# h3poteto/aws-global-accelerator-controller

Measured on NVIDIA H100. Metric: objects reconciled/sec at 10^6 Service+Ingress; change-set bit-exact vs Go ref, higher is better.
Workload: dtype u8/u32 (bytes and indices)

## Files before the change

aws-global-accelerator-controller_b200/csrc/gar_engine.cu:

```cuda

#include <cuda_runtime.h>
#include <unistd.h>

#include <cstdio>
#include <cstdlib>
#include <cstring>
#include <atomic>
#include <exception>
#include <functional>
#include <mutex>
#include <thread>
#include <string>
#include <vector>
#include <type_traits>
#include <utility>

#include "gar_pipeline.h"
#include "gar_shard.h"
#include "gar_delta.h"

#define GAR_VERSION_STRING "garecon 0.1.0 (sm_90a)"


template <class F>
__global__ void __launch_bounds__(256) k_for_each(const __grid_constant__ F f, u32 n) {
  u32 i = blockIdx.x * blockDim.x + threadIdx.x;
  if (i < n) f(i);
}

template <class F, int MINB>
__global__ void __launch_bounds__(256, MINB) k_for_each_warp(const __grid_constant__ F f, u32 n) {
  u32 i = blockIdx.x * blockDim.x + threadIdx.x;
  f(i, i < n);
}
__device__ __forceinline__ u32 smem_addr(const void *p) { return (u32)__cvta_generic_to_shared(p); }
__device__ __forceinline__ void mbar_init(u64 *bar, u32 count) {
  asm volatile("mbarrier.init.shared::cta.b64 [%0], %1;" ::"r"(smem_addr(bar)), "r"(count));
  asm volatile("fence.mbarrier_init.release.cluster;" ::: "memory");
}
__device__ __forceinline__ void mbar_expect_tx(u64 *bar, u32 bytes) {
  asm volatile("mbarrier.arrive.expect_tx.shared::cta.b64 _, [%0], %1;" ::"r"(smem_addr(bar)), "r"(bytes) : "memory");
}
__device__ __forceinline__ void tma_bulk_g2s(void *dst, const void *src, u32 bytes, u64 *bar) {
  asm volatile("cp.async.bulk.shared::cluster.global.mbarrier::complete_tx::bytes [%0], [%1], %2, [%3];" ::"r"(smem_addr(dst)), "l"(src), "r"(bytes),
               "r"(smem_addr(bar))
               : "memory");
}
__device__ __forceinline__ void mbar_wait(u64 *bar, u32 parity) {
  u32 done;
  do {
    asm volatile("{ .reg .pred p; mbarrier.try_wait.parity.shared::cta.b64 p, [%1], %2; selp.u32 %0, 1, 0, p; }" : "=r"(done) : "r"(smem_addr(bar)), "r"(parity) : "memory");
  } while (!done);
}
struct StagedView {
  const u8 *smem[2];
  const u8 *slab[2];
  u64 lo[2], hi[2];
  __device__ __forceinline__ Str operator()(int c, gar_str r) const {
    const u64 o = GAR_STR_OFF(r), n = GAR_STR_LEN(r);
    if (o >= lo[c] && o + n + 16 <= hi[c]) return Str{smem[c] + (o - lo[c]), (u32)n};
    return Str{slab[c] + o, (u32)n};
  }
};
template <class F>
__global__ void __launch_bounds__(256) k_for_each_staged(const __grid_constant__ F f, u32 n) {
  constexpr u32 STAGE_BYTES = F::kStageBytes;
  __shared__ alignas(128) u8 buf[F::kStageCols][STAGE_BYTES];
  __shared__ alignas(8) u64 bar;
  __shared__ u32 s_bytes[2];
  __shared__ u64 s_lo[2];
  const u32 r0 = blockIdx.x * blockDim.x, r1 = min(r0 + blockDim.x, n);
  if (threadIdx.x == 0) {
    mbar_init(&bar, 1);
    u32 total = 0;
    for (int c = 0; c < F::kStageCols; c++) {
      u64 lo = 0, hi = 0;
      u32 bytes = 0;
      const u8 *slab = f.stage_slab(c);
      if (f.stage_window(c, r0, r1, &lo, &hi) && hi > lo && (((uintptr_t)slab) & 15) == 0) {
        lo &= ~(u64)15;
        u64 span = ((hi - lo + 15) & ~(u64)15) + 16;
        if (span > STAGE_BYTES) span = STAGE_BYTES;
        bytes = (u32)span;
      }
      s_lo[c] = lo;
      s_bytes[c] = bytes;
      total += bytes;
    }
    mbar_expect_tx(&bar, total);
    for (int c = 0; c < F::kStageCols; c++)
      if (s_bytes[c]) tma_bulk_g2s(buf[c], f.stage_slab(c) + s_lo[c], s_bytes[c], &bar);
  }
  __syncthreads();
  StagedView view;
#pragma unroll
  for (int c = 0; c < 2; c++) {
    const bool on = c < F::kStageCols;
    view.smem[c] = on ? buf[c < F::kStageCols ? c : 0] : nullptr;
    view.slab[c] = on ? f.stage_slab(c) : nullptr;
    view.lo[c] = on ? s_lo[c] : 1;
    view.hi[c] = on ? s_lo[c] + s_bytes[c] : 0;
  }
  mbar_wait(&bar, 0);
  const u32 i = r0 + threadIdx.x;
  if (i < n) f.run(i, view);
}

template <class F>
__global__ void __launch_bounds__(256) k_for_each_dyn(const __grid_constant__ F f, const u32 *n_dev, u32 cap) {
  u32 n = *n_dev;
  if (n > cap) n = cap;
  u32 i = blockIdx.x * blockDim.x + threadIdx.x;
  if (i < n) f(i);
}
template <class F, int MINB>
__global__ void __launch_bounds__(256, MINB) k_for_each_warp_dyn(const __grid_constant__ F f, const u32 *n_dev, u32 cap) {
  u32 n = *n_dev;
  if (n > cap) n = cap;
  u32 i = blockIdx.x * blockDim.x + threadIdx.x;
  if (i < ((n + 31u) & ~31u)) f(i, i < n);
}
template <class... Fs>
struct FPack;
template <>
struct FPack<> {
  __device__ __forceinline__ void call(int, u32) const {}
};
template <class F, class... R>
struct FPack<F, R...> {
  F f;
  FPack<R...> rest;
  FPack(const F &f_, const R &...r) : f(f_), rest(r...) {}
  __device__ __forceinline__ void call(int k, u32 i) const {
    if (k == 0) f(i);
    else rest.call(k - 1, i);
  }
};
constexpr int MULTI_MAX = 8;
struct MultiRanges {
  u32 blk_end[MULTI_MAX], n[MULTI_MAX];
  int count;
};
template <class P>
__global__ void __launch_bounds__(256) k_for_each_multi(const __grid_constant__ P pack, const __grid_constant__ MultiRanges r) {
  int k = 0;
  while (k + 1 < r.count && blockIdx.x >= r.blk_end[k]) k++;
  u32 i = (blockIdx.x - (k ? r.blk_end[k - 1] : 0u)) * blockDim.x + threadIdx.x;
  if (i < r.n[k]) pack.call(k, i);
}

template <class F> struct MinBlocks { static constexpr int value = 2; };
template <> struct MinBlocks<FGaObj> { static constexpr int value = 4; };
template <> struct MinBlocks<FR53Pair> { static constexpr int value = 6; };
template <> struct MinBlocks<FR53Prepare> { static constexpr int value = 6; };

__global__ void k_fill32(u32 *p, u32 v, size_t n) {
  size_t i = (size_t)blockIdx.x * blockDim.x + threadIdx.x;
  size_t stride = (size_t)gridDim.x * blockDim.x;
  for (; i < n; i += stride) p[i] = v;
}

constexpr int SCAN_THREADS = 256;
constexpr int SCAN_ITEMS = 8;
constexpr int SCAN_TILE = SCAN_THREADS * SCAN_ITEMS;

__device__ __forceinline__ u32 warp_incl_scan(u32 v) {
  const unsigned lane = threadIdx.x & 31;
#pragma unroll
  for (int d = 1; d < 32; d <<= 1) {
    u32 t = __shfl_up_sync(0xffffffffu, v, d);
    if (lane >= (unsigned)d) v += t;
  }
  return v;
}
__device__ __forceinline__ u32 block_excl_scan(u32 v, u32 *total) {
  __shared__ u32 wsum[SCAN_THREADS / 32];
  __shared__ u32 wtot;
  const unsigned lane = threadIdx.x & 31, w = threadIdx.x >> 5;
  u32 inc = warp_incl_scan(v);
  if (lane == 31) wsum[w] = inc;
  __syncthreads();
  if (w == 0) {
    u32 s = lane < SCAN_THREADS / 32 ? wsum[lane] : 0;
    u32 si = warp_incl_scan(s);
    if (lane < SCAN_THREADS / 32) wsum[lane] = si - s;
    if (lane == SCAN_THREADS / 32 - 1) wtot = si;
  }
  __syncthreads();
  u32 r = wsum[w] + inc - v;
  *total = wtot;
  __syncthreads();
  return r;
}

__global__ void __launch_bounds__(SCAN_THREADS) k_scan_lookback(u32 *data, u32 n, unsigned long long *state, u32 *ticket) {
  __shared__ u32 s_tile, s_excl;
  if (threadIdx.x == 0) s_tile = atomicAdd(ticket, 1u);
  __syncthreads();
  const u32 tile = s_tile;
  const u32 base = tile * SCAN_TILE + threadIdx.x * SCAN_ITEMS;
  u32 v[SCAN_ITEMS];
  if (base + SCAN_ITEMS <= n) {
    const uint4 *q = reinterpret_cast<const uint4 *>(data + base);
    uint4 a = q[0], b = q[1];
    v[0] = a.x; v[1] = a.y; v[2] = a.z; v[3] = a.w;
    v[4] = b.x; v[5] = b.y; v[6] = b.z; v[7] = b.w;
  } else {
#pragma unroll
    for (int k = 0; k < SCAN_ITEMS; k++) v[k] = base + k < n ? data[base + k] : 0;
  }
  u32 s = 0;
#pragma unroll
  for (int k = 0; k < SCAN_ITEMS; k++) s += v[k];
  u32 total;
  u32 ex = block_excl_scan(s, &total);
  if (threadIdx.x < 32) {
    volatile unsigned long long *st = state;
    const unsigned lane = threadIdx.x;
    if (tile == 0) {
      if (lane == 0) {
        st[0] = (2ull << 62) | total;
        s_excl = 0;
      }
    } else {
      if (lane == 0) {
        st[tile] = (1ull << 62) | total;
        __threadfence();
      }
      u32 excl = 0;
      for (long long p = (long long)tile - 1;; p -= 32) {
        long long idx = p - (long long)lane;
        unsigned long long w = 2ull << 62;
        if (idx >= 0) {
          do {
            w = st[idx];
          } while ((w >> 62) == 0);
        }
        unsigned pm = __ballot_sync(0xffffffffu, (w >> 62) == 2);
        int first = __ffs(pm) - 1;
        u32 val = (first < 0 || (int)lane <= first) ? (u32)w : 0u;
#pragma unroll
        for (int off = 16; off > 0; off >>= 1) val += __shfl_down_sync(0xffffffffu, val, off);
        excl += val;
        if (first >= 0) break;
      }
      if (lane == 0) {
        st[tile] = (2ull << 62) | (u32)(excl + total);
        s_excl = excl;
      }
    }
  }
  __syncthreads();
  ex += s_excl;
  if (base + SCAN_ITEMS <= n) {
    uint4 a, b;
    a.x = ex; ex += v[0];
    a.y = ex; ex += v[1];
    a.z = ex; ex += v[2];
// ... 275 lines not shown
    for (int r = 0; r < 2; r++)
      for (int k = 0; k < GAR_SHARD_MAX_RANKS; k++) {
        if (peer_mapped[r][k]) cudaIpcCloseMemHandle(peer_ptr[r][k]);
        peer_mapped[r][k] = false;
        peer_ptr[r][k] = nullptr;
        peer_seen[r][k] = PeerHandle{};
      }
  }
  std::vector<HostResult *> free_results;
  float ms_h2d = 0;
  u32 launches = 0;
  u64 input_bytes = 0;
  bool timing = false;
  bool reprepare = false;
  bool no_orphans = false, allow_empty_cache = false;
  struct Mark {
    const char *name;
    cudaEvent_t a, b;
    u32 launches;
  };
  std::vector<Mark> marks;
  std::vector<cudaEvent_t> event_pool;
  size_t events_used = 0;
  int stage_depth = 0;
  u32 stage_launch0 = 0;
  std::vector<gar_stage_timing> last_timings;
  u64 last_counters[GAR_CTR_N] = {};
  cudaEvent_t new_event() {
    if (events_used == event_pool.size()) {
      cudaEvent_t ev;
      CK(cudaEventCreate(&ev));
      event_pool.push_back(ev);
    }
    return event_pool[events_used++];
  }
  void stage_begin(const char *name) {
    if (!timing || stage_depth++ > 0) return;
    Mark m{name, new_event(), new_event(), 0};
    CK(cudaEventRecord(m.a, stream));
    stage_launch0 = launches;
    marks.push_back(m);
  }
  void stage_end() {
    if (!timing || --stage_depth > 0) return;
    marks.back().launches = launches - stage_launch0;
    CK(cudaEventRecord(marks.back().b, stream));
  }

  void *dev_ensure(DBuf &b, size_t bytes) {
    bytes = (bytes + 255) & ~(size_t)255;
    if (b.cap < bytes) {
      if (capturing) throw CudaError{"internal: a buffer grew while a launch sequence was being recorded"};
      graph_drop();
      if (b.p) CK(cudaFree(b.p));
      b.p = nullptr;
      b.cap = 0;
      size_t want = bytes + bytes / 4;
      CK(cudaMalloc(&b.p, want));
      b.cap = want;
    }
    return b.p;
  }
  void *pin_ensure(DBuf &b, size_t bytes) {
    if (bytes < 64) bytes = 64;
    if (b.cap < bytes) {
      if (b.p) CK(cudaFreeHost(b.p));
      b.p = nullptr;
      b.cap = 0;
      size_t want = bytes + bytes / 4;
      CK(cudaMallocHost(&b.p, want));
      b.cap = want;
    }
    return b.p;
  }

  bool pack_tma = false;
  template <class F>
  void for_each(const char *name, u32 n, const F &f) {
    if (!n) return;
    stage_begin(name);
    if constexpr (std::is_same<F, FShPackRows>::value) {
      if (pack_tma) {
        k_shard_pack_rows<<<(n + 255) / 256, 256, 0, stream>>>(f, n);
        launches++;
        stage_end();
        return;
      }
    }
    k_for_each<F><<<(n + 255) / 256, 256, 0, stream>>>(f, n);
    launches++;
    stage_end();
  }
  template <class F>
  void for_each_warp(const char *name, u32 n, const F &f) {
    if (!n) return;
    stage_begin(name);
    k_for_each_warp<F, MinBlocks<F>::value><<<(n + 255) / 256, 256, 0, stream>>>(f, n);
    launches++;
    stage_end();
  }
  u32 hint_dport_cap = 0, hint_pair_cap = 0;
  u64 hint_ops_cap = 0;
  bool use_graphs = true;
  cudaGraphExec_t graph_exec = nullptr;
  u64 graph_sig = 0, seen_sig = 0;
  u32 graph_launches = 0, capture_launch0 = 0;
  bool capturing = false;
  void graph_drop() {
    if (graph_exec) cudaGraphExecDestroy(graph_exec);
    graph_exec = nullptr;
    graph_sig = seen_sig = 0;
  }
  int graph_begin(u64 sig) {
    if (!use_graphs || timing) return 0;
    if (graph_exec && graph_sig == sig) {
      CK(cudaGraphLaunch(graph_exec, stream));
      launches += graph_launches;
      return 2;
    }
    if (seen_sig != sig) {
      graph_drop();
      seen_sig = sig;
      return 0;
    }
    graph_drop();
    seen_sig = sig;
    CK(cudaStreamBeginCapture(stream, cudaStreamCaptureModeThreadLocal));
    capturing = true;
    capture_launch0 = launches;
    return 1;
  }
  void graph_end() {
    if (!capturing) return;
    capturing = false;
    cudaGraph_t g = nullptr;
    CK(cudaStreamEndCapture(stream, &g));
    cudaError_t ie = cudaGraphInstantiate(&graph_exec, g, 0);
    cudaGraphDestroy(g);
    if (ie != cudaSuccess) {
      graph_exec = nullptr;
      throw CudaError{std::string("cudaGraphInstantiate failed: ") + cudaGetErrorString(ie)};
    }
    graph_sig = seen_sig;
    graph_launches = launches - capture_launch0;
    CK(cudaGraphLaunch(graph_exec, stream));
  }
  bool staged_passes = true, staged_all = false;
  template <class F>
  void for_each_staged(const char *name, u32 n, const F &f) {
    if (!n) return;
    if (!staged_passes || !(F::kStageByDefault || staged_all)) return for_each(name, n, f);
    stage_begin(name);
    k_for_each_staged<F><<<(n + 255) / 256, 256, 0, stream>>>(f, n);
    launches++;
    stage_end();
  }
  template <class F>
  void for_each_dyn(const char *name, const u32 *n_dev, u32 cap, const F &f) {
    if (!cap) return;
    stage_begin(name);
    k_for_each_dyn<F><<<(cap + 255) / 256, 256, 0, stream>>>(f, n_dev, cap);
    launches++;
    stage_end();
  }
  template <class F>
  void for_each_warp_dyn(const char *name, const u32 *n_dev, u32 cap, const F &f) {
    if (!cap) return;
    stage_begin(name);
    k_for_each_warp_dyn<F, MinBlocks<F>::value><<<(cap + 255) / 256, 256, 0, stream>>>(f, n_dev, cap);
    launches++;
    stage_end();
  }
  template <class... Fs>
  void for_each_multi(const char *name, std::initializer_list<u32> ns, const Fs &...fs) {
    static_assert(sizeof...(Fs) <= MULTI_MAX, "too many functors for one fused launch");
    MultiRanges r{};
    u32 blocks = 0;
    for (u32 n : ns) {
      blocks += (n + 255) / 256;
      r.blk_end[r.count] = blocks;
      r.n[r.count] = n;
      r.count++;
    }
    if (!blocks) return;
    stage_begin(name);
    k_for_each_multi<FPack<Fs...>><<<blocks, 256, 0, stream>>>(FPack<Fs...>(fs...), r);
    launches++;
    stage_end();
  }
  void fill32(u32 *p, u32 v, size_t n) {
    if (!n) return;
    if (v == 0) {
      CK(cudaMemsetAsync(p, 0, n * 4, stream));
      return;
    }
    size_t blocks = (n + 255) / 256;
    if (blocks > 132 * 16) blocks = 132 * 16;
    k_fill32<<<(unsigned)blocks, 256, 0, stream>>>(p, v, n);
    launches++;
  }
  void copy32(u32 *dst, const u32 *src, size_t n) {
    if (n) CK(cudaMemcpyAsync(dst, src, n * 4, cudaMemcpyDeviceToDevice, stream));
  }
  void exclusive_scan(u32 *data, u32 n) {
    if (!n) return;
    stage_begin("exclusive_scan");
    u32 ntiles = (n + SCAN_TILE - 1) / SCAN_TILE;
    size_t sbytes = 8 * (size_t)(ntiles + 2);
    unsigned long long *state = (unsigned long long *)dev_ensure(d_scan_tiles, sbytes);
    CK(cudaMemsetAsync(state, 0, sbytes, stream));
    k_scan_lookback<<<ntiles, SCAN_THREADS, 0, stream>>>(data, n, state, (u32 *)(state + ntiles + 1));
    launches += 1;
    stage_end();
  }
  void sort_pairs(u32 *keys, u32 *vals, u32 *keys_alt, u32 *vals_alt, u32 n, int bits) {
    if (!n) return;
    stage_begin("radix_sort_pairs");
    u32 ntiles = (n + RS_TILE - 1) / RS_TILE;
    u32 *hist = (u32 *)dev_ensure(d_hist, 4 * (size_t)256 * ntiles + 16);
    u32 *ka = keys, *va = vals, *kb = keys_alt, *vb = vals_alt;
    int passes = (bits + 7) / 8;
    for (int p = 0; p < passes; p++) {
      k_radix_hist<<<ntiles, RS_THREADS, 0, stream>>>(ka, n, p * 8, hist, ntiles);
      launches++;
      exclusive_scan(hist, 256 * ntiles);
      k_radix_scatter<<<ntiles, RS_THREADS, 0, stream>>>(ka, va, kb, vb, n, p * 8, hist, ntiles);
      launches++;
      std::swap(ka, kb);
      std::swap(va, vb);
    }
    if (ka != keys) {
      CK(cudaMemcpyAsync(keys, ka, 4 * (size_t)n, cudaMemcpyDeviceToDevice, stream));
      CK(cudaMemcpyAsync(vals, va, 4 * (size_t)n, cudaMemcpyDeviceToDevice, stream));
    }
    stage_end();
  }
  void *ensure(int s, size_t bytes) { return dev_ensure(slot[s], bytes); }
  void download(void *dst, const void *src, size_t bytes) {
    CK(cudaMemcpyAsync(dst, src, bytes, cudaMemcpyDeviceToHost, stream));
    CK(cudaStreamSynchronize(stream));
  }
  DBuf dl_pin[2];
  cudaEvent_t dl_ev[2] = {};
  void download_start(int id, const void *src, size_t bytes) {
    void *p = pin_ensure(dl_pin[id], 64);
    if (!dl_ev[id]) CK(cudaEventCreateWithFlags(&dl_ev[id], cudaEventDisableTiming));
    CK(cudaMemcpyAsync(p, src, bytes, cudaMemcpyDeviceToHost, stream));
    CK(cudaEventRecord(dl_ev[id], stream));
  }
  void download_wait(int id, void *dst, size_t bytes) {
    CK(cudaEventSynchronize(dl_ev[id]));
    memcpy(dst, dl_pin[id].p, bytes);
  }
  void *out_derived(u32 n) { return dev_ensure(d_derived, 4 * (size_t)(n + 1)); }
  void *out_derived_keys(u32 n) { return dev_ensure(d_derived_keys, 4 * (size_t)(n + 1)); }
  void *out_dport_begin(u32 n) { return dev_ensure(d_dport_begin, 4 * (size_t)(n + 2)); }
  void *out_tok_code(u32 n) { return dev_ensure(d_tok_code, (size_t)n + 1); }
  void *out_tok_name(u32 n) { return dev_ensure(d_tok_name, 8 * (size_t)(n + 1)); }
  void *out_tok_region(u32 n) { return dev_ensure(d_tok_region, 8 * (size_t)(n + 1)); }
  void *out_dports(u64 n) { return dev_ensure(d_dports, 4 * (size_t)(n + 1)); }
  void *out_status_ga(u32 n) { return dev_ensure(d_status_ga, 4 * (size_t)(n + 1)); }
  void *out_status_r53(u32 n) { return dev_ensure(d_status_r53, 4 * (size_t)(n + 1)); }

  DBuf dset[DC_N], dscratch[DS_N];
  int o_set = 0;
  void upload(void *dst, const void *src, size_t bytes) {
    if (bytes) CK(cudaMemcpyAsync(dst, src, bytes, cudaMemcpyHostToDevice, stream));
  }
  void *delta_scratch(int k, size_t bytes) { return dev_ensure(dscratch[k], bytes); }
  void *delta_col(int c, size_t bytes) { return dev_ensure(o_set == 0 ? dset[c] : in[c], bytes); }
  void delta_swap() { o_set ^= 1; }
  u8 *delta_slab(u64 keep, u64 need) { return grow_slab(in[DC_N], keep, need); }
  DBuf aset[AC_N];
  bool a_alt[AC_N] = {};
  void *delta_actual_col(int c, size_t bytes) { return dev_ensure(a_alt[c] ? in[DC_N + 1 + c] : aset[c], bytes); }
  void delta_actual_swap(int c) { a_alt[c] = !a_alt[c]; }
  u8 *delta_actual_slab(u64 keep, u64 need) { return grow_slab(in[DC_N + 1 + AC_N], keep, need); }
  u8 *grow_slab(DBuf &b, u64 keep, u64 need) {
    if (b.cap < need + 16) {
      graph_drop();
      size_t want = (size_t)(need + need / 2 + 256) & ~(size_t)255;
      void *p = nullptr;
      CK(cudaMalloc(&p, want));
      if (keep) CK(cudaMemcpyAsync(p, b.p, keep, cudaMemcpyDeviceToDevice, stream));
      CK(cudaStreamSynchronize(stream));
      CK(cudaFree(b.p));
      b.p = p;
      b.cap = want;
    }
    return (u8 *)b.p;
  }
};


static void check_str_col(const char *name, const gar_str *col, size_t n, u64 slab_len) {
  if (n && !col) throw InvalidError{std::string(name) + " is NULL"};
  for (size_t i = 0; i < n; i++) {
    u64 off = GAR_STR_OFF(col[i]), len = GAR_STR_LEN(col[i]);
    if (off + len > slab_len) throw InvalidError{std::string(name) + ": string reference outside the slab"};
  }
}
static void check_csr(const char *name, const u32 *b, size_t nparents, size_t nchildren) {
  if (!b) throw InvalidError{std::string(name) + " is NULL"};
  if (b[0] != 0) throw InvalidError{std::string(name) + "[0] != 0"};
  for (size_t i = 0; i < nparents; i++)
    if (b[i + 1] < b[i]) throw InvalidError{std::string(name) + " is not monotone"};
// ... 899 lines not shown
```

aws-global-accelerator-controller_b200/csrc/gar_pipeline.h:

```cpp
#pragma once

#include <stdio.h>
#include <stdlib.h>

#include <initializer_list>

#include "gar_rows.h"

#if defined(__CUDA_ARCH__)
#define GAR_ATOMIC_ADD(p, v) atomicAdd((p), (v))
#else
#define GAR_ATOMIC_ADD(p, v) (*(p) += (v))
#endif


enum Slot {
  S_DERIVED, S_OFLAGS, S_OKEY_HASH, S_STAGE_GA, S_STAGE_R53, S_ANN_R53, S_ANN_NAME, S_ANN_TAGS, S_ANN_LISTEN, S_DPORT_BEGIN, S_DPORTS,
  S_TOK_CODE, S_TOK_NAME, S_TOK_REGION,
  S_ACC_FLAGS, S_ACC_OWNER_KEY, S_ACC_OWNER, S_ACC_THOST, S_ACC_MANAGED, S_ACC_OWNER_HASH, S_ACC_THOST_HASH, S_REC_NAME_HASH, S_VAL_KEY_HASH,
  S_REC_ZONE, S_VAL_REC, S_VAL_CLS, S_VAL_KEY, S_VAL_ORPHAN, S_VAL_LINK, S_ACC_DIGEST,
  S_R53_MODE, S_R53_ACC, S_R53_ACC_DNS, S_PAIR_BEGIN, S_PAIR_OBJ, S_PAIR_HN, S_PAIR_CODE, S_PAIR_ZONE, S_PAIR_REC,
  S_IX_LB, S_IX_OWNER = S_IX_LB + 3, S_IX_THOST = S_IX_OWNER + 3, S_IX_ZONE = S_IX_THOST + 3, S_IX_VAL = S_IX_ZONE + 3,
  S_IX_ALIAS = S_IX_VAL + 3, S_IX_OBJ = S_IX_ALIAS + 3, S_IX_OVN = S_IX_OBJ + 3,
  S_SORT_KEYS = S_IX_OVN + 3, S_SORT_VALS, S_SORT_KEYS_ALT, S_SORT_VALS_ALT, S_SORT_TAGS,
  S_COUNTS, S_STATUS_GA, S_STATUS_R53, S_OPS, S_ERRFLAG, S_IX_EG, S_IX_EG_ENT, S_IX_EG_PAD,
  S_VAL_OBJ, S_ACC_OBJ, S_OBJ_CANON, S_OWN_BEGIN, S_OWN_FILL, S_OWN_ENT, S_OWN_MULTI,
  S_IXA_BEGIN, S_IXA_FILL, S_IXA_ENT, S_IXA_MULTI, S_OVN_FILL, S_OVN_MULTI, S_LB_HASH, S_REC_FLAGS,
  S_NSLOTS
};


struct FClassify {
  DevTables T;
  Work W;
  u32 *derived_public;
  u8 *oflags;
  u32 *errflag;
  GAR_HD void operator()(u32 i) const {
    classify_object(T, W, i);
    W.obj_canon[i] = i;
    u32 dv = W.derived[i];
    if (dv & OBJ_KEY_BAD) GAR_ATOMIC_ADD(errflag, 1u);
    derived_public[i] = dv & 0xFFu;
  }
};
struct FTokenise {
  DevTables T;
  Work W;
  static constexpr int kStageCols = 1;
  static constexpr u32 kStageBytes = 24 * 1024;
  static constexpr bool kStageByDefault = true;
  GAR_HD void operator()(u32 i) const { tokenise_hostname(T, W, i); }
  GAR_HD const u8 *stage_slab(int) const { return T.o.slab; }
  GAR_HD bool stage_window(int, u32 r0, u32 r1, u64 *lo, u64 *hi) const {
    gar_str a = T.o.lbi_hostname[r0], b = T.o.lbi_hostname[r1 - 1];
    *lo = GAR_STR_OFF(a);
    *hi = GAR_STR_OFF(b) + GAR_STR_LEN(b);
    return true;
  }
  template <class View>
  GAR_HD void run(u32 i, const View &view) const { tokenise_hostname_at(T, W, i, view(0, T.o.lbi_hostname[i])); }
};
struct FDigestAccel {
  DevTables T;
  Work W;
  GAR_HD void operator()(u32 i) const { digest_accelerator(T, W, i); }
};
struct FExpand {
  const u32 *begin;
  u32 nparents;
  u32 *parent_of;
  GAR_HD void operator()(u32 c) const {
    u32 lo = 0, hi = nparents;
    while (hi - lo > 1) {
      u32 mid = (lo + hi) >> 1;
      if (begin[mid] <= c) lo = mid;
      else hi = mid;
    }
    parent_of[c] = lo;
  }
};
constexpr u32 REC_INLINE_VALUES = 32;
constexpr u32 REC_HUGE_VALUES = 4096;
struct DirectView {
  const u8 *slab;
  GAR_HD Str operator()(int, gar_str r) const { return mkstr(slab, r); }
};
struct FPrepareRecord {
  DevTables T;
  Work W;
  u32 *big, *huge;
  static constexpr int kStageCols = 2;
  static constexpr u32 kStageBytes = 16 * 1024;
  static constexpr bool kStageByDefault = true;
  GAR_HD const u8 *stage_slab(int) const { return T.a.slab; }
  GAR_HD bool stage_window(int c, u32 r0, u32 r1, u64 *lo, u64 *hi) const {
    if (c == 0) {
      gar_str a = T.a.rec_name[r0], b = T.a.rec_name[r1 - 1];
      *lo = GAR_STR_OFF(a);
      *hi = GAR_STR_OFF(b) + GAR_STR_LEN(b);
      return true;
    }
    u32 v0 = T.a.rec_val_begin[r0], v1 = T.a.rec_val_begin[r1];
    if (v1 == v0) return false;
    gar_str a = T.a.val_value[v0], b = T.a.val_value[v1 - 1];
    *lo = GAR_STR_OFF(a);
    *hi = GAR_STR_OFF(b) + GAR_STR_LEN(b);
    return true;
  }
  GAR_HD void operator()(u32 r) const { run(r, DirectView{T.a.slab}); }
  template <class View>
  GAR_HD void run(u32 r, const View &view) const {
    u32 lo = 0, hi = T.a.n_zones;
    while (hi - lo > 1) {
      u32 mid = (lo + hi) >> 1;
      if (T.a.zone_rec_begin[mid] <= r) lo = mid;
      else hi = mid;
    }
    W.rec_zone[r] = lo;
    const Str nm = view(0, T.a.rec_name[r]);
    const u64 nh = gar_hash(nm);
    W.rec_name_hash[r] = nh;
    W.rec_flags[r] = find_byte(nm, 0, '\\') < nm.n ? 1 : 0;
    if (T.a.rec_has_alias[r]) ix_count(W.hist[IX_ALIAS], key_hash_zoned_h(lo, nh));
    u32 v0 = T.a.rec_val_begin[r], v1 = T.a.rec_val_begin[r + 1];
    if (v1 - v0 > REC_INLINE_VALUES) {
      u32 *list = v1 - v0 > REC_HUGE_VALUES ? huge : big;
#if defined(__CUDA_ARCH__)
      list[1 + atomicAdd(list, 1u)] = r;
#else
      list[1 + list[0]++] = r;
#endif
      return;
    }
    for (u32 v = v0; v < v1; v++) {
      W.val_rec[v] = r;
      classify_value_at(T, W, v, view(1, T.a.val_value[v]));
    }
  }
};
constexpr u32 BIG_BLOCKS = 528;
struct FClassifyBigRecords {
  DevTables T;
  Work W;
  const u32 *big, *huge;
  GAR_HD void operator()(u32 i) const {
    const u32 blk = i >> 8, tid = i & 255u, nbig = big[0], nhuge = huge[0];
    for (u32 k = blk; k < nbig; k += BIG_BLOCKS) {
      u32 r = big[1 + k];
      for (u32 v = T.a.rec_val_begin[r] + tid; v < T.a.rec_val_begin[r + 1]; v += 256) {
        W.val_rec[v] = r;
        classify_value(T, W, v);
      }
    }
    for (u32 k = 0; k < nhuge; k++) {
      u32 r = huge[1 + k];
      for (u32 v = T.a.rec_val_begin[r] + i; v < T.a.rec_val_begin[r + 1]; v += BIG_BLOCKS * 256) {
        W.val_rec[v] = r;
        classify_value(T, W, v);
      }
    }
  }
};
struct FJsonCount {
  DevTables T;
  Work W;
  GAR_HD void operator()(u32 i) const {
    u32 n = 0;
    if (W.derived[i] & GAR_DV_PORTS_FROM_ANN) {
      u32 stk[GAR_JSON_STACK_WORDS];
      int c = json_listen_ports(mkstr(T.o.slab, W.ann_listen[i]), nullptr, stk);
      n = c < 0 ? 0u : (u32)c;
    }
    W.dport_begin[i] = n;
  }
};
struct FJsonWrite {
  DevTables T;
  Work W;
  GAR_HD void operator()(u32 i) const {
    if (!(W.derived[i] & GAR_DV_PORTS_FROM_ANN)) return;
    if (W.dport_begin[i + 1] == W.dport_begin[i] || W.dport_begin[i + 1] > W.dport_cap) return;
    u32 stk[GAR_JSON_STACK_WORDS];
    json_listen_ports(mkstr(T.o.slab, W.ann_listen[i]), W.dports + W.dport_begin[i], stk);
  }
};

struct FLbHash {
  DevTables T;
  Work W;
  GAR_HD void operator()(u32 i) const {
    u64 h = key_hash_lb(mkstr(T.a.slab, T.a.lb_region[i]), mkstr(T.a.slab, T.a.lb_name[i]));
    W.lb_hash[i] = h;
    ix_count(W.hist[IX_LB], h);
  }
};
struct FRowLb {
  DevTables T;
  Work W;
  GAR_HD bool make(u32 i, u64 *h, IdxEntry *e) const {
    *h = W.lb_hash[i];
    e->a0 = T.a.lb_state[i];
    e->a1 = 0;
    e->s0 = T.a.lb_name[i];
    e->s1 = T.a.lb_region[i];
    return true;
  }
};
struct FRowOwner {
  DevTables T;
  Work W;
  GAR_HD bool make(u32 i, u64 *h, IdxEntry *e) const {
    u32 fl = W.acc_flags[i];
    *h = W.acc_owner_hash[i];
    e->a0 = fl;
    e->a1 = 0;
    e->s0 = W.acc_owner_key[i];
    e->s1 = 0;
    return (fl & ACC_MINE) && (fl & ACC_OWNER_KEYED) && i < W.acc_guest_from;
  }
};
struct FRowThost {
  DevTables T;
  Work W;
  GAR_HD bool make(u32 i, u64 *h, IdxEntry *e) const {
    *h = W.acc_thost_hash[i];
    e->a0 = e->a1 = 0;
    e->s0 = W.acc_thost[i];
    e->s1 = T.a.acc_dns[i];
    return (W.acc_flags[i] & ACC_MINE) != 0 && (!W.sharded || i >= W.acc_guest_from);
  }
};
struct FRowZone {
  DevTables T;
  GAR_HD bool make(u32 i, u64 *h, IdxEntry *e) const {
    Str zn = mkstr(T.a.slab, T.a.zone_name[i]);
    bool valid = zn.n >= 1 && zn.p[zn.n - 1] == '.';
    *h = valid ? key_hash_str(substr(zn, 0, zn.n - 1)) : 0;
    e->a0 = e->a1 = 0;
    e->s0 = T.a.zone_name[i];
    e->s1 = 0;
    return valid;
  }
};
struct FZoneLenMask {
  DevTables T;
  Work W;
  unsigned long long *mask;
  GAR_HD void operator()(u32 z) const {
    Str zn = mkstr(T.a.slab, T.a.zone_name[z]);
    if (zn.n < 1 || zn.p[zn.n - 1] != '.') return;
    ix_count(W.hist[IX_ZONE], key_hash_str(substr(zn, 0, zn.n - 1)));
    u32 b = zn.n - 1 < 255 ? zn.n - 1 : 255;
#if defined(__CUDA_ARCH__)
    atomicOr(&mask[b >> 6], 1ull << (b & 63));
#else
    mask[b >> 6] |= 1ull << (b & 63);
#endif
  }
};
struct FRowVal {
  DevTables T;
  Work W;
  GAR_HD bool make(u32 v, u64 *h, IdxEntry *e) const {
    u32 cls = W.val_cls[v];
    *h = W.val_key_hash[v];
    if (cls == VAL_NOT_OWNER) return false;
    u32 rec = W.val_rec[v];
    u32 kind = (cls & VAL_OWNER_INGRESS) ? 1u : 0u;
    u32 bs = (W.rec_flags[rec] & 1) ? VALNAME_HAS_BACKSLASH : 0u;
    e->a0 = rec;
    e->a1 = W.rec_zone[rec] | bs | (kind << 31);
    e->s0 = W.val_key[v];
    e->s1 = T.a.rec_name[rec];
    return true;
  }
};
struct FRowAlias {
  DevTables T;
  Work W;
  GAR_HD bool make(u32 r, u64 *h, IdxEntry *e) const {
    *h = key_hash_zoned_h(W.rec_zone[r], W.rec_name_hash[r]);
    e->a0 = W.rec_zone[r];
    e->a1 = T.a.rec_type[r];
    e->s0 = T.a.rec_name[r];
    e->s1 = T.a.rec_alias_dns[r];
    return T.a.rec_has_alias[r] != 0;
  }
};
struct FRowObj {
  DevTables T;
  Work W;
  GAR_HD bool make(u32 i, u64 *h, IdxEntry *e) const {
    gar_str ns = T.o.obj_ns[i];
    *h = W.okey_hash[i];
    e->a0 = T.o.obj_kind[i];
    e->a1 = 0;
    e->s0 = GAR_STR(GAR_STR_OFF(ns), GAR_STR_LEN(ns) + 1 + GAR_STR_LEN(T.o.obj_name[i]));
    e->s1 = 0;
    return !(W.derived[i] & OBJ_KEY_BAD);
  }
};
struct FRowOvn {
  DevTables T;
  Work W;
  GAR_HD bool make(u32 v, u64 *h, IdxEntry *e) const {
    u32 rec = W.val_rec[v];
    *h = key_hash_zoned_h(W.rec_zone[rec], W.rec_name_hash[rec]);
    e->a0 = rec;
    e->a1 = W.rec_zone[rec];
    e->s0 = T.a.rec_name[rec];
    e->s1 = T.a.val_value[v];
    return W.val_orphan[v] != 0;
  }
};

constexpr u32 IDX_SMALL_BUCKET = 48;
struct CanonHook {
  u32 *canon;
  const u8 *slab;
  u32 b0, b1;
  GAR_HD void operator()(u32 b, const IdxEntry *ent, u32 lo, u32 m) const {
    if (canon && b >= b0 && b < b1) canon_bucket(ent, lo, m, slab, canon);
  }
};
template <class RowF>
struct FIdxRows {
  RowF rowf;
  u32 *keys, *vals;
  IdxEntry *tmp;
  u32 *counts;
  u32 mask, nb;
  GAR_HD void operator()(u32 i) const {
    u64 h = 0;
    IdxEntry e;
    bool valid = rowf.make(i, &h, &e);
    u32 k = valid ? hash_bucket(h, mask) : nb;
    keys[i] = k;
    if (vals) vals[i] = i;
    if (valid) {
      e.tag = hash_tag(h);
      e.row = i;
      tmp[i] = e;
      GAR_ATOMIC_ADD(&counts[k], 1u);
    }
  }
};
struct FIdxPlace {
  const u32 *keys;
  u32 *cursor;
  const IdxEntry *tmp;
  IdxEntry *ent;
  u32 nb;
  GAR_HD void operator()(u32 i) const {
    u32 k = keys[i];
    if (k == nb) return;
#if defined(__CUDA_ARCH__)
    u32 pos = atomicAdd(&cursor[k], 1u);
#else
    u32 pos = cursor[k]++;
#endif
    ent[pos] = tmp[i];
  }
};
struct FIdxOrder {
  const u32 *begin;
  IdxEntry *ent;
  u32 *overflow;
  CanonHook canon;
  GAR_HD void operator()(u32 b) const {
    u32 lo = begin[b], m = begin[b + 1] - lo;
    if (m < 2) return;
    if (m > IDX_SMALL_BUCKET) {
      GAR_ATOMIC_ADD(overflow, 1u);
      return;
    }
    for (u32 k = 1; k < m; k++) {
      IdxEntry x = ent[lo + k];
      u32 j = k;
      while (j > 0 && ent[lo + j - 1].row > x.row) {
        ent[lo + j] = ent[lo + j - 1];
        j--;
      }
      if (j != k) ent[lo + j] = x;
    }
    canon(b, ent, lo, m);
  }
};
struct FIdxGather {
  const u32 *vals;
  const u32 *nvalid;
  const IdxEntry *tmp;
  IdxEntry *ent;
  GAR_HD void operator()(u32 p) const {
    if (p < *nvalid) ent[p] = tmp[vals[p]];
  }
};
struct FIdxCanon {
  const u32 *begin;
  const IdxEntry *ent;
  CanonHook canon;
  GAR_HD void operator()(u32 b) const {
    const u32 lo = begin[b], m = begin[b + 1] - lo;
    if (m >= 2) canon(b, ent, lo, m);
  }
};
template <class RowF>
struct FIdxPlaceDirect {
  RowF rowf;
  u32 *cursor;
  IdxEntry *ent;
  u32 mask;
  GAR_HD void operator()(u32 i) const {
    u64 h = 0;
    IdxEntry e;
    if (!rowf.make(i, &h, &e)) return;
    const u32 k = hash_bucket(h, mask);
#if defined(__CUDA_ARCH__)
    const u32 pos = atomicAdd(&cursor[k], 1u);
#else
    const u32 pos = cursor[k]++;
#endif
    e.tag = hash_tag(h);
    e.row = i;
    ent[pos] = e;
  }
};
struct FIdxMultiList {
  const u32 *begin;
  u32 *multi;
  GAR_HD void operator()(u32 b) const {
    const bool m = begin[b + 1] - begin[b] >= 2;
#if defined(__CUDA_ARCH__)
    const unsigned active = __activemask();
    const unsigned votes = __ballot_sync(active, m);
    if (!m) return;
    const unsigned lane = threadIdx.x & 31u;
    const int leader = __ffs(votes) - 1;
    u32 base = 0;
    if ((int)lane == leader) base = atomicAdd(multi, (u32)__popc(votes));
    base = __shfl_sync(votes, base, leader);
    multi[1 + base + __popc(votes & ((1u << lane) - 1u))] = b;
#else
    if (m) multi[1 + multi[0]++] = b;
#endif
  }
};
struct FIdxOrderMulti {
  const u32 *begin;
  IdxEntry *ent;
  const u32 *multi;
  u32 *overflow;
  CanonHook canon;
  GAR_HD void operator()(u32 t) const {
    const u32 b = multi[1 + t];
    const u32 lo = begin[b], m = begin[b + 1] - lo;
    if (m > IDX_SMALL_BUCKET) {
      GAR_ATOMIC_ADD(overflow, 1u);
      return;
    }
    for (u32 k = 1; k < m; k++) {
      IdxEntry x = ent[lo + k];
      u32 j = k;
      while (j > 0 && ent[lo + j - 1].row > x.row) {
        ent[lo + j] = ent[lo + j - 1];
        j--;
      }
      if (j != k) ent[lo + j] = x;
    }
    canon(b, ent, lo, m);
  }
};
enum FlagWord { FW_BAD_KEYS = 0, FW_IDX_OVERFLOW = 1, FW_NDPORTS = 2, FW_NPAIRS = 3, FW_SEC0 = 4 , FW_WORDS = 16 };
struct FGatherFinal {
  const u32 *src;
  u32 idx[5];
  const u32 *npairs;
  u32 *flags;
  GAR_HD void operator()(u32 k) const {
    if (k < 5) flags[FW_SEC0 + k] = src[idx[k]];
    else if (npairs) flags[FW_NPAIRS] = *npairs;
  }
};
struct FGather5 {
  const u32 *src;
  u32 idx[5];
  const u32 *extra;
  u32 *dst;
  GAR_HD void operator()(u32 k) const { dst[k] = k < 5 ? src[idx[k]] : *extra; }
};
#define GAR_RETRY_WITH_RADIX 1000
#define GAR_REFUSE_EMPTY_CACHE 1001
struct FGatherHeader {
  const u32 *ndports;
  u32 *flags;
  GAR_HD void operator()(u32) const { flags[FW_NDPORTS] = *ndports; }
};
struct FValueJoins {
  DevTables T;
  Work W;
  GAR_HD void operator()(u32 v) const {
    link_value_alias(T, W, v);
    resolve_value(T, W, v);
  }
};
struct FResolveValue {
  DevTables T;
  Work W;
  GAR_HD void operator()(u32 v) const { resolve_value(T, W, v); }
};
struct FResolveAccel {
  DevTables T;
  Work W;
  GAR_HD void operator()(u32 a) const { resolve_accel(T, W, a); }
};
GAR_HD IdxEntry own_entry(const DevTables &T, const Work &W, u32 x) {
  IdxEntry e;
  e.tag = e.a0 = e.a1 = 0;
  e.s0 = e.s1 = 0;
  if (x < T.a.n_accels) {
    e.row = x;
    return e;
  }
  const u32 v = x - T.a.n_accels, rec = W.val_rec[v];
  const ValLink l = W.val_link[v];
  e.tag = l.alias_row;
  e.row = v;
  e.a0 = rec;
  e.a1 = W.rec_zone[rec] | ((W.rec_flags[rec] & 1) ? VALNAME_HAS_BACKSLASH : 0u);
  e.s0 = l.alias_dns;
  e.s1 = T.a.rec_name[rec];
  return e;
}
GAR_HD u32 own_segment(const DevTables &T, const Work &W, u32 x) {
  const u32 nacc = T.a.n_accels;
  const u32 o = x < nacc ? W.acc_obj[x] : W.val_obj[x - nacc];
  return o == GAR_NONE ? 2 * T.o.n_objects : 2 * o + (x < nacc ? 0u : 1u);
}
struct FOwnPlace {
  DevTables T;
  Work W;
  u32 *cursor;
  IdxEntry *ent;
  u32 x0;
  GAR_HD void operator()(u32 i) const {
    const u32 x = x0 + i, k = own_segment(T, W, x);
    if (k == 2 * T.o.n_objects) return;
#if defined(__CUDA_ARCH__)
    const u32 pos = atomicAdd(&cursor[k], 1u);
#else
    const u32 pos = cursor[k]++;
#endif
    ent[pos] = own_entry(T, W, x);
  }
};
struct FOwnKeys {
  DevTables T;
  Work W;
  u32 *keys, *vals;
  GAR_HD void operator()(u32 x) const {
    keys[x] = own_segment(T, W, x);
    vals[x] = x;
  }
};
struct FOwnGather {
  DevTables T;
  Work W;
  const u32 *vals;
  const u32 *total;
  IdxEntry *ent;
  GAR_HD void operator()(u32 p) const {
    if (p < *total) ent[p] = own_entry(T, W, vals[p]);
  }
};

struct CountLayout {
  u32 n, nacc, nrec, nval;
  GAR_HD u32 ga_obj(u32 i) const { return i; }
  GAR_HD u32 ga_orph(u32 a) const { return n + a; }
  GAR_HD u32 r53_obj(u32 i) const { return n + nacc + i; }
  GAR_HD u32 base0() const { return 2 * n + nacc; }
  GAR_HD u32 base1() const { return 2 * n + nacc + nrec; }
  GAR_HD u32 total() const { return 2 * n + nacc + nrec + nval; }
};
constexpr u32 OPS_STAGE_CAP = 4;
struct FGaObj {
  DevTables T;
  Work W;
  u32 *counts;
  gar_op *stage;
  u32 *status;
  const u32 *rows;
  GAR_HD void operator()(u32 t, bool valid) const {
    u32 i = (rows && valid) ? rows[t] : t;
    OpSink s{stage + (size_t)t * OPS_STAGE_CAP, 0, OPS_STAGE_CAP};
    u32 st = ga_reconcile(T, W, i, valid, s);
    if (valid) {
      status[t] = st;
      counts[t] = s.n;
    }
  }
};
struct FR53Obj {
  DevTables T;
  Work W;
  u32 *counts;
  gar_op *stage;
  u32 *status;
  const u32 *rows;
  GAR_HD void operator()(u32 t, bool valid) const {
    u32 i = (rows && valid) ? rows[t] : t;
    OpSink s{stage + (size_t)t * OPS_STAGE_CAP, 0, OPS_STAGE_CAP};
    u32 prev = (valid && W.r53_mode[i] == R53_MODE_DONE) ? status[t] : 0;
    u32 st = r53_combine(T, W, i, t, valid, prev, s);
    if (valid) {
      status[t] = st;
      counts[t] = s.n;
    }
  }
};
struct FR53Prepare {
  DevTables T;
  Work W;
  u32 *status;
  const u32 *rows;
  GAR_HD void operator()(u32 t, bool valid) const { r53_prepare(T, W, (rows && valid) ? rows[t] : t, t, valid, status); }
};
struct FR53FillPairs {
  DevTables T;
  Work W;
  const u32 *rows;
  GAR_HD void operator()(u32 t) const { r53_fill_pairs(T, W, rows ? rows[t] : t, t); }
};
struct FR53Pair {
  DevTables T;
  Work W;
  GAR_HD void operator()(u32 p, bool valid) const { r53_pair(T, W, p, valid); }
};
struct DelKeys {
  const u8 *kind;
  const gar_str *key;
  const u8 *slab;
};
struct FDelKeyGa {
  DevTables T;
  Work W;
  DelKeys D;
  u32 *counts;
  gar_op *ops;
  u32 cap;
  GAR_HD void operator()(u32 k) const {
    u32 kind = D.kind[k];
    Str key = mkstr(D.slab, D.key[k]);
    if (ops && counts[k + 1] > cap) return;
    OpSink s{ops ? ops + counts[k] : nullptr, 0, 0xFFFFFFFFu};
    OwnerIter it = owner_open(W, key_hash_kinded(kind, key), key);
    for (u32 acc; (acc = owner_next(T, W, kind, it)) != GAR_NONE;) put_delete_chain(T, s, GAR_NONE, 0, acc);
    if (!ops) counts[k] = s.n;
  }
};
struct FDelKeyR53 {
  DevTables T;
  Work W;
  DelKeys D;
  u32 *counts;
  gar_op *ops;
  u32 cap;
  GAR_HD void operator()(u32 k) const {
    u32 kind = D.kind[k];
    Str key = mkstr(D.slab, D.key[k]);
    if (ops && counts[k + 1] > cap) return;
    OpSink s{ops ? ops + counts[k] : nullptr, 0, 0xFFFFFFFFu};
    Owned ow;
    owned_collect(T, W, key_hash_kinded(kind, key), kind, key, ow);
    r53_cleanup(T, W, GAR_NONE, 0, ow, s);
    if (!ops) counts[k] = s.n;
  }
};
struct FRowKnownEg {
  gar_bindings b;
  GAR_HD bool make(u32 i, u64 *h, IdxEntry *e) const {
    *h = gar_hash(mkstr(b.slab, b.known_eg_arn[i]));
    e->a0 = e->a1 = 0;
    e->s0 = b.known_eg_arn[i];
    e->s1 = 0;
    return true;
  }
};
struct FEgb {
  DevTables T;
  Work W;
  DevBindings B;
  u32 *counts;
  gar_op *ops;
  u32 *status;
  u32 cap;
  GAR_HD void operator()(u32 k) const {
    if (ops && counts[k + 1] > cap) return;
    OpSink s{ops ? ops + counts[k] : nullptr, 0, 0xFFFFFFFFu};
    u32 st = egb_reconcile(T, W, B, k, s);
    if (ops) status[k] = st;
    else counts[k] = s.n;
  }
};
struct FGatherDerived {
  const u32 *derived, *rows;
  u32 *out;
  GAR_HD void operator()(u32 t) const { out[t] = derived[rows[t]] & 0xFFu; }
};
struct FCompactOps {
  DevTables T;
  Work W;
  const u32 *scanned;
  const gar_op *stage;
  gar_op *ops;
  u32 ctrl;
  const u32 *rows;
  u32 cap;
  GAR_HD void operator()(u32 t, bool valid) const {
    u32 i = (rows && valid) ? rows[t] : t;
    u32 off = 0, c = 0;
    if (valid) {
      off = scanned[t];
      c = scanned[t + 1] - off;
      if (off > cap || c > cap - off) c = 0;
      if (c <= OPS_STAGE_CAP)
        for (u32 k = 0; k < c; k++) ops[off + k] = stage[(size_t)t * OPS_STAGE_CAP + k];
    }
    bool redo = valid && c > OPS_STAGE_CAP;
    if (GAR_ANY(redo)) {
      OpSink s{ops + off, 0, redo ? c : 0u};
      if (ctrl == GAR_CTRL_GA) ga_reconcile(T, W, i, redo, s);
      else r53_reconcile(T, W, i, redo, s);
    }
  }
};
struct FGaOrphan {
  DevTables T;
  Work W;
  CountLayout L;
  u32 *counts;
  gar_op *ops;
  u32 cap;
  GAR_HD void operator()(u32 a) const {
    if (ops && counts[L.ga_orph(a) + 1] == counts[L.ga_orph(a)]) return;
    if (ops && counts[L.ga_orph(a) + 1] > cap) return;
    OpSink s{ops ? ops + counts[L.ga_orph(a)] : nullptr, 0, 0xFFFFFFFFu};
    ga_orphan(T, W, a, s);
    if (!ops) counts[L.ga_orph(a)] = s.n;
  }
};
struct FR53OrphanAlias {
  DevTables T;
  Work W;
  CountLayout L;
  u32 *counts;
  gar_op *ops;
  u32 cap;
  GAR_HD void operator()(u32 r) const {
    if (!ops) {
      OpSink s{nullptr, 0, 0};
      r53_orphan_alias(T, W, r, s);
      counts[L.base0() + r] = s.n;
      return;
    }
    if (counts[L.base0() + r + 1] == counts[L.base0() + r]) return;
    if (counts[L.total()] > cap) return;
    u32 z = W.rec_zone[r];
    u32 zv = T.a.rec_val_begin[T.a.zone_rec_begin[z]];
    u32 off = counts[L.base0()] + (counts[L.base1() + zv] - counts[L.base1()]) + (counts[L.base0() + r] - counts[L.base0()]);
    OpSink s{ops + off, 0, 0xFFFFFFFFu};
    r53_orphan_alias(T, W, r, s);
  }
};
struct FR53OrphanValue {
  DevTables T;
  Work W;
  CountLayout L;
  u32 *counts;
  gar_op *ops;
  u32 cap;
  GAR_HD void operator()(u32 v) const {
    if (!ops) {
      counts[L.base1() + v] = W.val_orphan[v];
      return;
    }
    if (!W.val_orphan[v] || counts[L.total()] > cap) return;
    u32 r = W.val_rec[v];
    u32 z = W.rec_zone[r];
    u32 rend = T.a.zone_rec_begin[z + 1];
    u32 off = counts[L.base0()] + (counts[L.base0() + rend] - counts[L.base0()]) + (counts[L.base1() + v] - counts[L.base1()]);
    gar_op o;
    o.head = GAR_OP_HEAD(GAR_OP_R53_DELETE_RECORD, GAR_CTRL_R53, 0);
    o.obj = GAR_NONE;
    o.sub = 1;
    o.a0 = z;
    o.a1 = r;
    o.a2 = v;
    ops[off] = o;
  }
};


struct DiffCounts {
  u64 n_ops;
  u64 section_begin[GAR_N_SECTIONS + 1];
  u64 n_dports;
  u32 bad_keys;
};

GAR_HD u32 next_pow2(u32 x) {
  u32 p = 1;
  while (p < x) p <<= 1;
  return p;
}
inline int ilog2(u32 p) {
  int b = 0;
  while ((1u << b) < p) b++;
  return b;
}

template <class B>
struct Pipeline {
  B &be;
  DevTables T;
  Work W{};
  bool force_radix = false;
  explicit Pipeline(B &b, const DevTables &t) : be(b), T(t) {}

  template <class RowF>
  HashIdx build_index(int slot, u32 nrows, u32 load, RowF rowf, u32 *overflow, bool force_radix, CanonHook canon = {}) {
    u32 nb = next_pow2(nrows / load < 16 ? 16 : nrows / load);
    u32 *keys = (u32 *)be.ensure(S_SORT_KEYS, sizeof(u32) * (size_t)(nrows + 1));
    u32 *vals = (u32 *)be.ensure(S_SORT_VALS, sizeof(u32) * (size_t)(nrows + 1));
    IdxEntry *tmp = (IdxEntry *)be.ensure(S_SORT_TAGS, sizeof(IdxEntry) * (size_t)(nrows + 1));
    u32 *begin = (u32 *)be.ensure(slot + 0, sizeof(u32) * (size_t)(nb + 2));
    IdxEntry *ent = (IdxEntry *)be.ensure(slot + 1, sizeof(IdxEntry) * (size_t)(nrows + 1));
    be.fill32(begin, 0, nb + 2);
    if (nrows) be.for_each("idx_rows", nrows, FIdxRows<RowF>{rowf, keys, force_radix ? vals : nullptr, tmp, begin, nb - 1, nb});
    be.exclusive_scan(begin, nb + 2);
    if (nrows && !force_radix) {
      u32 *cursor = (u32 *)be.ensure(S_SORT_KEYS_ALT, sizeof(u32) * (size_t)(nb + 1));
      be.copy32(cursor, begin, nb);
      be.for_each("idx_place", nrows, FIdxPlace{keys, cursor, tmp, ent, nb});
      be.for_each("idx_order", nb, FIdxOrder{begin, ent, overflow, canon});
    } else if (nrows) {
      u32 *keys2 = (u32 *)be.ensure(S_SORT_KEYS_ALT, sizeof(u32) * (size_t)(nrows + 1));
      u32 *vals2 = (u32 *)be.ensure(S_SORT_VALS_ALT, sizeof(u32) * (size_t)(nrows + 1));
      be.sort_pairs(keys, vals, keys2, vals2, nrows, ilog2(nb) + 1);
      be.for_each("idx_gather", nrows, FIdxGather{vals, begin + nb, tmp, ent});
      if (canon.canon) be.for_each("idx_order", nb, FIdxCanon{begin, ent, canon});
    }
    return HashIdx{begin, ent, nb - 1};
  }

  bool prepared = false;
  u64 n_dports = 0;
  u32 *errflag = nullptr;

  u32 acc_guest_from = 0xFFFFFFFFu;
  u32 sharded = 0;
  bool orphan_sweep = true;
  bool allow_empty_cache = false;

  void alloc_obj_work() {
    const u32 n = T.o.n_objects, nlbi = T.o.n_lbi;
    W.derived = (u32 *)be.ensure(S_DERIVED, 4 * (size_t)(n + 1));
    W.okey_hash = (u64 *)be.ensure(S_OKEY_HASH, 8 * (size_t)(n + 1));
    W.ann_r53 = (gar_str *)be.ensure(S_ANN_R53, 8 * (size_t)(n + 1));
    W.ann_name = (gar_str *)be.ensure(S_ANN_NAME, 8 * (size_t)(n + 1));
    W.ann_tags = (gar_str *)be.ensure(S_ANN_TAGS, 8 * (size_t)(n + 1));
    W.ann_listen = (gar_str *)be.ensure(S_ANN_LISTEN, 8 * (size_t)(n + 1));
    W.dport_begin = (u32 *)be.out_dport_begin(n);
    W.tok_code = (u8 *)be.out_tok_code(nlbi);
    W.tok_name = (gar_str *)be.out_tok_name(nlbi);
    W.tok_region = (gar_str *)be.out_tok_region(nlbi);
    W.r53_mode = (u8 *)be.ensure(S_R53_MODE, (size_t)n + 1);
    W.r53_acc = (u32 *)be.ensure(S_R53_ACC, 4 * (size_t)(n + 1));
    W.r53_acc_dns = (gar_str *)be.ensure(S_R53_ACC_DNS, 8 * (size_t)(n + 1));
    W.obj_canon = (u32 *)be.ensure(S_OBJ_CANON, 4 * (size_t)(n + 1));
  }
  CanonHook canon_hook(u32 b0, u32 b1) const { return CanonHook{W.obj_canon, T.o.slab, b0, b1}; }
  void alloc_work() {
    const u32 nacc = T.a.n_accels, nrec = T.a.n_records, nval = T.a.n_values;
    alloc_obj_work();
    W.acc_flags = (u32 *)be.ensure(S_ACC_FLAGS, 4 * (size_t)(nacc + 1));
    W.acc_owner_key = (gar_str *)be.ensure(S_ACC_OWNER_KEY, 8 * (size_t)(nacc + 1));
    W.acc_owner = (gar_str *)be.ensure(S_ACC_OWNER, 8 * (size_t)(nacc + 1));
    W.acc_thost = (gar_str *)be.ensure(S_ACC_THOST, 8 * (size_t)(nacc + 1));
    W.acc_managed = (gar_str *)be.ensure(S_ACC_MANAGED, 8 * (size_t)(nacc + 1));
    W.acc_owner_hash = (u64 *)be.ensure(S_ACC_OWNER_HASH, 8 * (size_t)(nacc + 1));
    W.acc_thost_hash = (u64 *)be.ensure(S_ACC_THOST_HASH, 8 * (size_t)(nacc + 1));
    W.rec_name_hash = (u64 *)be.ensure(S_REC_NAME_HASH, 8 * (size_t)(nrec + 1));
    W.val_key_hash = (u64 *)be.ensure(S_VAL_KEY_HASH, 8 * (size_t)(nval + 1));
    W.rec_zone = (u32 *)be.ensure(S_REC_ZONE, 4 * (size_t)(nrec + 1));
    W.val_rec = (u32 *)be.ensure(S_VAL_REC, 4 * (size_t)(nval + 1));
    W.val_cls = (u8 *)be.ensure(S_VAL_CLS, nval + 1);
    W.val_key = (gar_str *)be.ensure(S_VAL_KEY, 8 * (size_t)(nval + 1));
    W.val_orphan = (u8 *)be.ensure(S_VAL_ORPHAN, nval + 1);
    W.val_obj = (u32 *)be.ensure(S_VAL_OBJ, 4 * (size_t)(nval + 1));
    W.acc_obj = (u32 *)be.ensure(S_ACC_OBJ, 4 * (size_t)(nacc + 1));
    W.val_link = (ValLink *)be.ensure(S_VAL_LINK, sizeof(ValLink) * (size_t)(nval + 1));
    W.acc_digest = (AccDigest *)be.ensure(S_ACC_DIGEST, sizeof(AccDigest) * (size_t)(nacc + 1));
    W.lb_hash = (u64 *)be.ensure(S_LB_HASH, 8 * (size_t)(T.a.n_lbs + 1));
    W.rec_flags = (u8 *)be.ensure(S_REC_FLAGS, (size_t)nrec + 1);
    for (int k = 0; k < IX_N; k++) W.hist[k] = IxHist{nullptr, 0};
    W.pair_cap = 0;
    W.dport_cap = 0;
    errflag = (u32 *)be.ensure(S_ERRFLAG, 256);
    be.fill32(errflag, 0, FW_WORDS);
    W.acc_guest_from = acc_guest_from;
    W.sharded = sharded;
  }
  void stage1() {
    const u32 n = T.o.n_objects, nlbi = T.o.n_lbi, nacc = T.a.n_accels, nrec = T.a.n_records, nval = T.a.n_values;
    u32 *derived_public = (u32 *)be.out_derived(n);
    if (n) be.for_each("classify_objects", n, FClassify{T, W, derived_public, nullptr, errflag});
    if (nlbi) be.for_each_staged("tokenise_hostnames", nlbi, FTokenise{T, W});
    if (nacc) be.for_each("digest_accelerators", nacc, FDigestAccel{T, W});
    if (T.a.n_lbs) be.for_each("hash_load_balancers", T.a.n_lbs, FLbHash{T, W});
    {
      unsigned long long *zm = (unsigned long long *)(errflag + 16 + 8);
      be.fill32((u32 *)zm, 0, 8);
      if (T.a.n_zones) be.for_each("zone_len_mask", T.a.n_zones, FZoneLenMask{T, W, zm});
      W.zone_len_mask = (const u64 *)zm;
    }
    if (nrec) {
      u32 *big = (u32 *)be.ensure(S_SORT_KEYS, 4 * (size_t)(nval / REC_INLINE_VALUES + 2));
      u32 *huge = (u32 *)be.ensure(S_SORT_VALS, 4 * (size_t)(nval / REC_HUGE_VALUES + 2));
      be.fill32(big, 0, 1);
      be.fill32(huge, 0, 1);
      be.for_each_staged("prepare_records", nrec, FPrepareRecord{T, W, big, huge});
      if (nval > REC_INLINE_VALUES) be.for_each("prepare_records", BIG_BLOCKS * 256, FClassifyBigRecords{T, W, big, huge});
    }
  }
  struct IxPlan {
    u32 off[IX_N] = {}, nb[IX_N] = {}, rows[IX_N] = {};
    bool want[IX_N] = {};
    u32 total_nb = 0;
    u64 total_rows = 0;
  };
  IxPlan planA;
  u32 *ixa_begin = nullptr, *ixa_fill = nullptr, *ixa_multi = nullptr;
  IdxEntry *ixa_ent = nullptr;
  u32 ovn_nb = 0;
  void arm_group_a(u32 want_mask) {
    const u32 rows[IX_N] = {T.a.n_lbs, T.a.n_accels, T.a.n_accels, T.a.n_zones, T.a.n_values, T.a.n_records, T.o.n_objects, 0};
    const u32 load[IX_N] = {1, 1, 1, 1, 1, 2, 1, 8};
    planA = IxPlan{};
    for (int k = 0; k < IX_OVN; k++) {
      planA.want[k] = (want_mask >> k) & 1u;
      if (!planA.want[k]) continue;
      planA.rows[k] = rows[k];
      planA.nb[k] = next_pow2(rows[k] / load[k] < 16 ? 16 : rows[k] / load[k]);
      planA.off[k] = planA.total_nb;
      planA.total_nb += planA.nb[k];
      planA.total_rows += rows[k];
    }
    ixa_begin = (u32 *)be.ensure(S_IXA_BEGIN, 4 * (size_t)(planA.total_nb + 2));
    be.fill32(ixa_begin, 0, (size_t)planA.total_nb + 2);
    for (int k = 0; k < IX_OVN; k++)
      if (planA.want[k]) W.hist[k] = IxHist{ixa_begin + planA.off[k], planA.nb[k] - 1};
  }
  HashIdx group_a_index(int k) const { return HashIdx{ixa_begin + planA.off[k], ixa_ent, planA.nb[k] - 1}; }
  template <class RowF>
  FIdxPlaceDirect<RowF> placer(int k, RowF rowf) const {
    return FIdxPlaceDirect<RowF>{rowf, ixa_fill + planA.off[k], ixa_ent, planA.nb[k] - 1};
  }
  void finish_group_a() {
    u32 *overflow = errflag + FW_IDX_OVERFLOW;
    be.exclusive_scan(ixa_begin, planA.total_nb + 1);
    ixa_fill = (u32 *)be.ensure(S_IXA_FILL, 4 * (size_t)(planA.total_nb + 1));
    ixa_ent = (IdxEntry *)be.ensure(S_IXA_ENT, sizeof(IdxEntry) * (size_t)(planA.total_rows + 1));
    const u32 multi_cap = (u32)(planA.total_rows / 2 + 1);
    ixa_multi = (u32 *)be.ensure(S_IXA_MULTI, 4 * (size_t)(multi_cap + 2));
    be.copy32(ixa_fill, ixa_begin, (size_t)planA.total_nb + 1);
    be.fill32(ixa_multi, 0, 1);
    const IxPlan &P = planA;
    auto n = [&](int k) { return P.want[k] ? P.rows[k] : 0u; };
    be.for_each_multi("idx_place", {n(IX_LB), n(IX_THOST), n(IX_ZONE), n(IX_ALIAS), n(IX_OBJ), P.total_nb},
                      placer(IX_LB, FRowLb{T, W}), placer(IX_THOST, FRowThost{T, W}), placer(IX_ZONE, FRowZone{T}),
                      placer(IX_ALIAS, FRowAlias{T, W}), placer(IX_OBJ, FRowObj{T, W}), FIdxMultiList{ixa_begin, ixa_multi});
    const CanonHook canon = P.want[IX_OBJ] ? canon_hook(P.off[IX_OBJ], P.off[IX_OBJ] + P.nb[IX_OBJ]) : CanonHook{};
    be.for_each_dyn("idx_order", ixa_multi, multi_cap, FIdxOrderMulti{ixa_begin, ixa_ent, ixa_multi, overflow, canon});
    if (P.want[IX_LB]) W.ix_lb = group_a_index(IX_LB);
    if (P.want[IX_THOST]) W.ix_thost = group_a_index(IX_THOST);
    if (P.want[IX_ZONE]) W.ix_zone = group_a_index(IX_ZONE);
    if (P.want[IX_ALIAS]) W.ix_alias = group_a_index(IX_ALIAS);
    if (P.want[IX_OBJ]) W.ix_obj = group_a_index(IX_OBJ);
  }
  void resolve_owners(bool link_aliases) {
    const u32 n = T.o.n_objects, nacc = T.a.n_accels, nval = T.a.n_values, nseg = 2 * n;
    u32 *overflow = errflag + FW_IDX_OVERFLOW;
    W.own_begin = (u32 *)be.ensure(S_OWN_BEGIN, 4 * (size_t)(nseg + 2));
    be.fill32(W.own_begin, 0, (size_t)nseg + 1);
    u32 *ovn = nullptr;
    if (!force_radix) {
      ovn_nb = next_pow2(nval / 8 < 16 ? 16 : nval / 8);
      ovn = (u32 *)be.ensure(S_IX_OVN + 0, 4 * (size_t)(ovn_nb + 2));
      be.fill32(ovn, 0, (size_t)ovn_nb + 2);
      W.hist[IX_OVN] = IxHist{ovn, ovn_nb - 1};
    } else {
      W.hist[IX_OVN] = IxHist{nullptr, 0};
    }
    if (link_aliases) be.for_each_multi("value_joins", {nval, nacc}, FValueJoins{T, W}, FResolveAccel{T, W});
    else be.for_each_multi("resolve_owners", {nval, nacc}, FResolveValue{T, W}, FResolveAccel{T, W});
    be.exclusive_scan(W.own_begin, nseg + 1);
    IdxEntry *own = (IdxEntry *)be.ensure(S_OWN_ENT, sizeof(IdxEntry) * ((size_t)nacc + nval + 1));
    if (!force_radix) {
      be.exclusive_scan(ovn, ovn_nb + 1);
      u32 *ovn_cursor = (u32 *)be.ensure(S_OVN_FILL, 4 * (size_t)(ovn_nb + 1));
      IdxEntry *ovn_ent = (IdxEntry *)be.ensure(S_IX_OVN + 1, sizeof(IdxEntry) * (size_t)(nval + 1));
      u32 *ovn_multi = (u32 *)be.ensure(S_OVN_MULTI, 4 * (size_t)(nval / 2 + 3));
      u32 *own_cursor = (u32 *)be.ensure(S_OWN_FILL, 4 * (size_t)(nseg + 1));
      const u32 own_multi_cap = (u32)(((u64)nacc + nval) / 2 + 1);
      u32 *own_multi = (u32 *)be.ensure(S_OWN_MULTI, 4 * (size_t)(own_multi_cap + 2));
      be.copy32(ovn_cursor, ovn, (size_t)ovn_nb + 1);
      be.copy32(own_cursor, W.own_begin, (size_t)nseg + 1);
      be.fill32(ovn_multi, 0, 1);
      be.fill32(own_multi, 0, 1);
      be.for_each_multi("idx_place", {nval, ovn_nb, nacc, nval, nseg}, FIdxPlaceDirect<FRowOvn>{FRowOvn{T, W}, ovn_cursor, ovn_ent, ovn_nb - 1},
                        FIdxMultiList{ovn, ovn_multi}, FOwnPlace{T, W, own_cursor, own, 0}, FOwnPlace{T, W, own_cursor, own, nacc},
                        FIdxMultiList{W.own_begin, own_multi});
      be.for_each_dyn("idx_order", ovn_multi, nval / 2 + 1, FIdxOrderMulti{ovn, ovn_ent, ovn_multi, overflow});
      be.for_each_dyn("idx_order", own_multi, own_multi_cap, FIdxOrderMulti{W.own_begin, own, own_multi, overflow});
      W.ix_ovn = HashIdx{ovn, ovn_ent, ovn_nb - 1};
    } else {
      const u32 nx = nacc + nval;
      u32 *keys = (u32 *)be.ensure(S_SORT_KEYS, 4 * (size_t)(nx + 1));
      u32 *vals = (u32 *)be.ensure(S_SORT_VALS, 4 * (size_t)(nx + 1));
      u32 *keys2 = (u32 *)be.ensure(S_SORT_KEYS_ALT, 4 * (size_t)(nx + 1));
      u32 *vals2 = (u32 *)be.ensure(S_SORT_VALS_ALT, 4 * (size_t)(nx + 1));
      if (nx) {
        be.for_each("own_keys", nx, FOwnKeys{T, W, keys, vals});
        be.sort_pairs(keys, vals, keys2, vals2, nx, ilog2(nseg + 1) + 1);
        be.for_each("own_gather", nx, FOwnGather{T, W, vals, W.own_begin + nseg, own});
      }
      W.ix_ovn = build_index(S_IX_OVN, nval, 8, FRowOvn{T, W}, overflow, true);
    }
    W.own = own;
    owners_stale = false;
  }
  bool owner_indexes = false;
  void build_owner_indexes() {
    if (owner_indexes) return;
    u32 *overflow = errflag + FW_IDX_OVERFLOW;
    W.ix_owner = build_index(S_IX_OWNER, T.a.n_accels, 1, FRowOwner{T, W}, overflow, force_radix);
    W.ix_val = build_index(S_IX_VAL, T.a.n_values, 1, FRowVal{T, W}, overflow, force_radix);
    owner_indexes = true;
  }

  void prepare_route() {
    alloc_work();
    arm_group_a(1u << IX_ALIAS);
    stage1();
    finish_group_a();
  }
  void prepare_directory() {
    alloc_work();
    arm_group_a((1u << IX_LB) | (1u << IX_THOST));
    if (T.o.n_lbi) be.for_each("tokenise_hostnames", T.o.n_lbi, FTokenise{T, W});
    if (T.a.n_accels) be.for_each("digest_accelerators", T.a.n_accels, FDigestAccel{T, W});
    if (T.a.n_lbs) be.for_each("hash_load_balancers", T.a.n_lbs, FLbHash{T, W});
    finish_group_a();
  }

  u32 dport_cap = 0, pair_cap = 0;
  u64 ops_cap = 0;
  bool tiny_caps = false;
  int prepare() {
    const u32 n = T.o.n_objects, nacc = T.a.n_accels, nzone = T.a.n_zones, nrec = T.a.n_records;
    alloc_work();
    if (!force_radix) arm_group_a((1u << IX_LB) | (1u << IX_THOST) | (1u << IX_ZONE) | (1u << IX_ALIAS) | (1u << IX_OBJ));
    stage1();
    listen_ports();

    u32 *overflow = errflag + FW_IDX_OVERFLOW;
    if (!force_radix) {
      finish_group_a();
    } else {
      W.ix_lb = build_index(S_IX_LB, T.a.n_lbs, 1, FRowLb{T, W}, overflow, true);
      W.ix_thost = build_index(S_IX_THOST, nacc, 1, FRowThost{T, W}, overflow, true);
      W.ix_zone = build_index(S_IX_ZONE, nzone, 1, FRowZone{T}, overflow, true);
      W.ix_alias = build_index(S_IX_ALIAS, nrec, 2, FRowAlias{T, W}, overflow, true);
      W.ix_obj = build_index(S_IX_OBJ, n, 1, FRowObj{T, W}, overflow, true, canon_hook(0, 0xFFFFFFFFu));
    }
    resolve_owners(true);
    obj_stale = false;
    owner_indexes = false;
    return GAR_OK;
  }
  void listen_ports() {
    const u32 n = T.o.n_objects;
    be.fill32(W.dport_begin, 0, (size_t)n + 1);
    if (n) be.for_each("listen_ports_count", n, FJsonCount{T, W});
    be.exclusive_scan(W.dport_begin, n + 1);
    be.for_each("gather_header", 1, FGatherHeader{W.dport_begin + n, errflag});
    if (dport_cap < n / 2 + 1024 && !(tiny_caps && dport_cap)) dport_cap = tiny_caps ? 1 : n / 2 + 1024;
    W.dport_cap = dport_cap;
    W.dports = (i32 *)be.out_dports(dport_cap);
    if (n) be.for_each("listen_ports_write", n, FJsonWrite{T, W});
  }

  bool obj_stale = false, owners_stale = false;
  void prepare_objects() {
    const u32 n = T.o.n_objects, nlbi = T.o.n_lbi;
    alloc_obj_work();
    be.fill32(errflag, 0, FW_WORDS);
    W.hist[IX_OBJ] = IxHist{nullptr, 0};
    u32 *derived_public = (u32 *)be.out_derived(n);
    if (n) be.for_each("classify_objects", n, FClassify{T, W, derived_public, nullptr, errflag});
    if (nlbi) be.for_each_staged("tokenise_hostnames", nlbi, FTokenise{T, W});
    listen_ports();
    W.ix_obj = build_index(S_IX_OBJ, n, 1, FRowObj{T, W}, errflag + FW_IDX_OVERFLOW, force_radix, canon_hook(0, 0xFFFFFFFFu));
    obj_stale = false;
    owners_stale = true;
  }
  int index_objects() {
    for (int attempt = 0; attempt < 2; attempt++) {
      if (!prepared) prepare();
      else if (obj_stale) prepare_objects();
      prepared = true;
      u32 fl[FW_WORDS];
      be.download(fl, errflag, sizeof(fl));
      if (fl[FW_BAD_KEYS]) return GAR_E_INVALID;
      if (fl[FW_IDX_OVERFLOW] && !force_radix) {
        force_radix = true;
        prepared = false;
        continue;
      }
      return GAR_OK;
    }
    return GAR_E_STATE;
  }

  u64 n_pairs = 0;
  void r53_relational(u32 slots, const u32 *rows, u32 *st_r53) {
    W.pair_begin = (u32 *)be.ensure(S_PAIR_BEGIN, 4 * (size_t)(slots + 2));
    be.fill32(W.pair_begin, 0, (size_t)slots + 1);
    if (slots) be.for_each_warp("r53_prepare", slots, FR53Prepare{T, W, st_r53, rows});
    be.exclusive_scan(W.pair_begin, slots + 1);
    if (pair_cap < slots + slots / 2 + 1024 && !(tiny_caps && pair_cap)) pair_cap = tiny_caps ? 1 : slots + slots / 2 + 1024;
    W.pair_cap = pair_cap;
    W.pair_obj = (u32 *)be.ensure(S_PAIR_OBJ, 4 * (size_t)(pair_cap + 1));
    W.pair_hn = (gar_str *)be.ensure(S_PAIR_HN, 8 * (size_t)(pair_cap + 1));
    W.pair_code = (u8 *)be.ensure(S_PAIR_CODE, (size_t)pair_cap + 1);
    W.pair_zone = (u32 *)be.ensure(S_PAIR_ZONE, 4 * (size_t)(pair_cap + 1));
    W.pair_rec = (u32 *)be.ensure(S_PAIR_REC, 4 * (size_t)(pair_cap + 1));
    if (slots) {
      be.for_each("r53_fill_pairs", slots, FR53FillPairs{T, W, rows});
      be.for_each_warp_dyn("r53_pairs", W.pair_begin + slots, pair_cap, FR53Pair{T, W});
    }
  }

  template <class OpsAlloc>
  int decide_all(OpsAlloc ops_alloc) {
    const u32 n = T.o.n_objects, nacc = T.a.n_accels, nrec = T.a.n_records, nval = T.a.n_values;
    CountLayout L{n, nacc, nrec, nval};
    u32 *counts = (u32 *)be.ensure(S_COUNTS, 4 * (size_t)(L.total() + 2));
    be.fill32(counts, 0, (size_t)L.total() + 1);
    gar_op *stage_ga = (gar_op *)be.ensure(S_STAGE_GA, sizeof(gar_op) * ((size_t)n * OPS_STAGE_CAP + 1));
    gar_op *stage_r53 = (gar_op *)be.ensure(S_STAGE_R53, sizeof(gar_op) * ((size_t)n * OPS_STAGE_CAP + 1));
    u32 *st_ga = (u32 *)be.out_status_ga(n);
    u32 *st_r53 = (u32 *)be.out_status_r53(n);
    if (n) be.for_each_warp("ga_objects", n, FGaObj{T, W, counts + L.ga_obj(0), stage_ga, st_ga, nullptr});
    r53_relational(n, nullptr, st_r53);
    if (n) be.for_each_warp("r53_objects", n, FR53Obj{T, W, counts + L.r53_obj(0), stage_r53, st_r53, nullptr});
    if (orphan_sweep)
      be.for_each_multi("orphans_count", {nacc, nrec, nval}, FGaOrphan{T, W, L, counts, nullptr, 0}, FR53OrphanAlias{T, W, L, counts, nullptr, 0},
                        FR53OrphanValue{T, W, L, counts, nullptr, 0});
    be.exclusive_scan(counts, L.total() + 1);
    be.for_each("gather_section_begins", 6, FGatherFinal{counts, {0, L.ga_orph(0), L.r53_obj(0), L.base0(), L.total()}, W.pair_begin + n, errflag});

    const u64 est = tiny_caps ? 1 : (u64)n + nacc / 8 + 1024;
    if (ops_cap < est) ops_cap = est;
    gar_op *ops = (gar_op *)ops_alloc(ops_cap);
    const u32 cap = ops_cap > 0xFFFFFFF0ull ? 0xFFFFFFF0u : (u32)ops_cap;
    if (n) be.for_each_warp("ga_objects_compact", n, FCompactOps{T, W, counts + L.ga_obj(0), stage_ga, ops, GAR_CTRL_GA, nullptr, cap});
    if (n) be.for_each_warp("r53_objects_compact", n, FCompactOps{T, W, counts + L.r53_obj(0), stage_r53, ops, GAR_CTRL_R53, nullptr, cap});
    if (orphan_sweep)
      be.for_each_multi("orphans_emit", {nacc, nrec, nval}, FGaOrphan{T, W, L, counts, ops, cap}, FR53OrphanAlias{T, W, L, counts, ops, cap},
                        FR53OrphanValue{T, W, L, counts, ops, cap});
    return GAR_OK;
  }

  template <class OpsAlloc>
  int decide_keys(const u32 *rows, u32 m, DelKeys D, u32 nd, OpsAlloc ops_alloc) {
    const u32 total = 2 * m + 2 * nd;
    u32 *counts = (u32 *)be.ensure(S_COUNTS, 4 * (size_t)(total + 2));
    be.fill32(counts, 0, (size_t)total + 1);
    u32 *c_ga = counts, *c_gad = counts + m, *c_r53 = counts + m + nd, *c_r53d = counts + 2 * m + nd;
    gar_op *stage_ga = (gar_op *)be.ensure(S_STAGE_GA, sizeof(gar_op) * ((size_t)m * OPS_STAGE_CAP + 1));
    gar_op *stage_r53 = (gar_op *)be.ensure(S_STAGE_R53, sizeof(gar_op) * ((size_t)m * OPS_STAGE_CAP + 1));
    u32 *st_ga = (u32 *)be.out_status_ga(m);
    u32 *st_r53 = (u32 *)be.out_status_r53(m);
    u32 *derived_out = (u32 *)be.out_derived_keys(m);
    if (nd) build_owner_indexes();
    if (m) {
      be.for_each("gather_derived", m, FGatherDerived{W.derived, rows, derived_out});
      be.for_each_warp("ga_objects", m, FGaObj{T, W, c_ga, stage_ga, st_ga, rows});
    }
    if (nd) be.for_each("ga_deleted_keys_count", nd, FDelKeyGa{T, W, D, c_gad, nullptr, 0});
    r53_relational(m, rows, st_r53);
    if (m) be.for_each_warp("r53_objects", m, FR53Obj{T, W, c_r53, stage_r53, st_r53, rows});
    if (nd) be.for_each("r53_deleted_keys_count", nd, FDelKeyR53{T, W, D, c_r53d, nullptr, 0});
    be.exclusive_scan(counts, total + 1);
    be.for_each("gather_section_begins", 6, FGatherFinal{counts, {0, m, m + nd, 2 * m + nd, total}, W.pair_begin + m, errflag});
    const u64 est = tiny_caps ? 1 : 2 * (u64)m + 4 * (u64)nd + 256;
    if (ops_cap < est) ops_cap = est;
    gar_op *ops = (gar_op *)ops_alloc(ops_cap);
    const u32 cap = ops_cap > 0xFFFFFFF0ull ? 0xFFFFFFF0u : (u32)ops_cap;
    if (m) be.for_each_warp("ga_objects_compact", m, FCompactOps{T, W, c_ga, stage_ga, ops, GAR_CTRL_GA, rows, cap});
    if (nd) be.for_each("ga_deleted_keys_emit", nd, FDelKeyGa{T, W, D, c_gad, ops, cap});
    if (m) be.for_each_warp("r53_objects_compact", m, FCompactOps{T, W, c_r53, stage_r53, ops, GAR_CTRL_R53, rows, cap});
    if (nd) be.for_each("r53_deleted_keys_emit", nd, FDelKeyR53{T, W, D, c_r53d, ops, cap});
    return GAR_OK;
  }

  template <class OpsAlloc>
  int decide_bindings(const gar_bindings &b, OpsAlloc ops_alloc) {
    u32 *overflow = errflag + FW_IDX_OVERFLOW;
    const u32 nb = b.n_bindings;
    DevBindings DB{b, build_index(S_IX_EG, b.n_known_egs, 1, FRowKnownEg{b}, overflow, force_radix)};
    u32 *counts = (u32 *)be.ensure(S_COUNTS, 4 * (size_t)(nb + 2));
    be.fill32(counts, 0, (size_t)nb + 1);
    u32 *st = (u32 *)be.out_status_ga(nb);
    if (nb) be.for_each("egb_count", nb, FEgb{T, W, DB, counts, nullptr, nullptr, 0});
    be.exclusive_scan(counts, nb + 1);
    be.for_each("gather_section_begins", 6, FGatherFinal{counts, {0, nb, nb, nb, nb}, nullptr, errflag});
    const u64 est = tiny_caps ? 1 : 4 * (u64)nb + 256;
    if (ops_cap < est) ops_cap = est;
    gar_op *ops = (gar_op *)ops_alloc(ops_cap);
    const u32 cap = ops_cap > 0xFFFFFFF0ull ? 0xFFFFFFF0u : (u32)ops_cap;
    if (nb) be.for_each("egb_emit", nb, FEgb{T, W, DB, counts, ops, st, cap});
    return GAR_OK;
  }

  template <class DecideF>
  int run_with(DiffCounts *dc, bool full, DecideF decide) {
    for (int attempt = 0; attempt < 8; attempt++) {
      u64 sig = 0;
      if (full) {
        sig = hmix(hmix(prepared ? (obj_stale || owners_stale ? 9 : 1) : 2, force_radix ? 3 : 4), hmix(hmix(dport_cap, pair_cap), ops_cap));
        sig = hmix(sig, hmix(orphan_sweep ? 5 : 6, tiny_caps ? 7 : 8)) | 1;
      }
      const int g = full ? be.graph_begin(sig) : 0;
      int rc = GAR_OK;
      if (g != 2) {
        if (!prepared) rc = prepare();
        else if (obj_stale) prepare_objects();
        if (rc == GAR_OK && owners_stale) resolve_owners(false);
        if (rc == GAR_OK) rc = decide();
      }
      prepared = true;
      if (full) be.graph_end();
      if (rc != GAR_OK) return rc;
      u32 fl[FW_WORDS];
      be.download(fl, errflag, sizeof(fl));
      if (fl[FW_BAD_KEYS]) return GAR_E_INVALID;
      if (fl[FW_IDX_OVERFLOW] && !force_radix) {
        force_radix = true;
        prepared = false;
        continue;
      }
      if (fl[FW_NDPORTS] > dport_cap) {
        dport_cap = fl[FW_NDPORTS] + fl[FW_NDPORTS] / 8 + 16;
        prepared = false;
        continue;
      }
      if (fl[FW_NPAIRS] > pair_cap) {
        pair_cap = fl[FW_NPAIRS] + fl[FW_NPAIRS] / 8 + 16;
        continue;
      }
      const u64 nops = fl[FW_SEC0 + 4];
      if (nops > ops_cap) {
        ops_cap = nops + nops / 8 + 16;
        continue;
      }
      n_dports = fl[FW_NDPORTS];
      n_pairs = fl[FW_NPAIRS];
      for (int k = 0; k < 5; k++) dc->section_begin[k] = fl[FW_SEC0 + k];
      dc->n_ops = nops;
      dc->n_dports = full ? n_dports : 0;
      if (full && T.o.n_objects == 0 && !sharded && !allow_empty_cache && nops != 0) return GAR_REFUSE_EMPTY_CACHE;
      return GAR_OK;
    }
    return GAR_E_STATE;
  }
  template <class OpsAlloc>
  int run(DiffCounts *dc, OpsAlloc ops_alloc) {
    return run_with(dc, true, [&] { return decide_all(ops_alloc); });
  }
  template <class OpsAlloc>
  int run_keys(const u32 *rows, u32 m, DelKeys D, u32 nd, DiffCounts *dc, OpsAlloc ops_alloc) {
    return run_with(dc, false, [&] { return decide_keys(rows, m, D, nd, ops_alloc); });
  }
  template <class OpsAlloc>
  int run_bindings(const gar_bindings &b, DiffCounts *dc, OpsAlloc ops_alloc) {
    return run_with(dc, false, [&] { return decide_bindings(b, ops_alloc); });
  }
};
```

aws-global-accelerator-controller_b200/csrc/gar_rows.h:

```cpp
#pragma once

#include "gar_common.h"
#include "gar_json.h"


struct DevTables {
  gar_objects o;
  gar_actual a;
  const u8 *cluster;
  u32 cluster_len;
};

enum {
  OBJ_HAS_NAME_ANN = 1u << 8,
  OBJ_HAS_TAGS_ANN = 1u << 9,
  OBJ_KEY_BAD = 1u << 10,
};

enum {
  ACC_MINE = 1u << 0,
  ACC_OWNER_KEYED = 1u << 1,
  ACC_OWNER_INGRESS = 1u << 2,
  ACC_OWNER_3PART = 1u << 3,
  ACC_HAS_MANAGED = 1u << 4, ACC_HAS_OWNER = 1u << 5, ACC_HAS_THOST = 1u << 6,
};

enum {
  R53_MODE_DONE = 0,
  R53_MODE_PAIRS = 1,
  R53_MODE_OBJECT = 2,
};
enum { PAIR_IN_SYNC = 0, PAIR_CREATE = 1, PAIR_UPSERT = 2, PAIR_NO_ZONE = 3,
       PAIR_REPEAT = 4 };
#define VALNAME_HAS_BACKSLASH (1u << 30)

enum { VAL_NOT_OWNER = 0, VAL_OWNER_SERVICE = 1, VAL_OWNER_INGRESS = 2, VAL_OWNER_3PART = 4 };

struct alignas(64) AccDigest {
  u32 flags;
  u32 lis;
  u32 eg;
  u32 pr_begin;
  u32 ep_begin;
  u16 n_ports, n_eps;
  i32 port0, port1;
  gar_str name;
  gar_str thost;
  gar_str owner_key;
  gar_str ep0;
};
enum {
  ACCD_ENABLED = 1u << 8,
  ACCD_MANAGED_TRUE = 1u << 9,
  ACCD_LIS_NONE = 1u << 10, ACCD_LIS_MANY = 1u << 11,
  ACCD_LIS_UDP = 1u << 12,
  ACCD_EG_NONE = 1u << 13, ACCD_EG_MANY = 1u << 14,
};
struct alignas(16) ValLink {
  u32 alias_row, pad;
  gar_str alias_dns;
};

enum IxId { IX_LB, IX_OWNER, IX_THOST, IX_ZONE, IX_VAL, IX_ALIAS, IX_OBJ, IX_OVN, IX_N };
struct IxHist {
  u32 *cnt;
  u32 mask;
};
#if defined(__CUDA_ARCH__)
#define GAR_HIST_ADD(p) atomicAdd((p), 1u)
#else
#define GAR_HIST_ADD(p) (++*(p))
#endif
GAR_HD void ix_count(const IxHist &h, u64 key_hash) {
  if (h.cnt) GAR_HIST_ADD(&h.cnt[(u32)key_hash & h.mask]);
}

struct Work {
  IxHist hist[IX_N];
  u64 *lb_hash;
  u8 *rec_flags;
  u32 pair_cap;
  u32 dport_cap;
  u32 *derived;
  u64 *okey_hash;
  gar_str *ann_r53;
  gar_str *ann_name;
  gar_str *ann_tags;
  gar_str *ann_listen;
  u32 *dport_begin;
  i32 *dports;
  u8 *tok_code;
  gar_str *tok_name, *tok_region;
  u32 *acc_flags;
  gar_str *acc_owner_key;
  gar_str *acc_owner;
  gar_str *acc_thost;
  gar_str *acc_managed;
  AccDigest *acc_digest;
  u64 *acc_owner_hash;
  u64 *acc_thost_hash;
  u32 *rec_zone;
  u64 *rec_name_hash;
  u32 *val_rec;
  u8 *val_cls;
  gar_str *val_key;
  u64 *val_key_hash;
  u8 *val_orphan;
  ValLink *val_link;
  u32 acc_guest_from;
  u32 sharded;
  u32 *val_obj;
  u32 *acc_obj;
  u32 *obj_canon;
  u32 *own_begin;
  const IdxEntry *own;
  u8 *r53_mode;
  u32 *r53_acc;
  gar_str *r53_acc_dns;
  u32 *pair_begin;
  u32 *pair_obj;
  gar_str *pair_hn;
  u8 *pair_code;
  u32 *pair_zone;
  u32 *pair_rec;
  HashIdx ix_lb;
  HashIdx ix_owner;
  HashIdx ix_thost;
  HashIdx ix_zone;
  const u64 *zone_len_mask;
  HashIdx ix_val;
  HashIdx ix_alias;
  HashIdx ix_obj;
  HashIdx ix_ovn;
};

GAR_HD bool acc_in_owner_index(const Work &W, u32 a, u32 fl) { return (fl & ACC_MINE) && (fl & ACC_OWNER_KEYED) && a < W.acc_guest_from; }
GAR_HD bool acc_in_thost_index(const Work &W, u32 a, u32 fl) { return (fl & ACC_MINE) != 0 && (!W.sharded || a >= W.acc_guest_from); }


GAR_HD u64 key_hash_kinded(u32 kind, Str nsname) { return hmix(kind + 1, gar_hash(nsname)); }
GAR_HD u64 key_hash_lb(Str region, Str name) { return hmix(gar_hash(region), gar_hash(name)); }
GAR_HD u64 key_hash_zoned_h(u32 zone, u64 name_hash) { return hmix((u64)zone + 0x100, name_hash); }
GAR_HD u64 key_hash_zoned(u32 zone, Str name) { return key_hash_zoned_h(zone, gar_hash(name)); }
GAR_HD u64 key_hash_str(Str s) { return gar_hash(s); }

GAR_HD Str object_key(const DevTables &T, u32 i) {
  gar_str ns = T.o.obj_ns[i], nm = T.o.obj_name[i];
  return Str{T.o.slab + GAR_STR_OFF(ns), GAR_STR_LEN(ns) + 1 + GAR_STR_LEN(nm)};
}
GAR_HD bool object_key_ok(const DevTables &T, u32 i) {
  gar_str ns = T.o.obj_ns[i], nm = T.o.obj_name[i];
  u64 sep = GAR_STR_OFF(ns) + GAR_STR_LEN(ns);
  return GAR_STR_OFF(nm) == sep + 1 && sep < T.o.slab_len && T.o.slab[sep] == '/';
}


#define ANN_PREFIX "aws-global-accelerator-controller.h3poteto.dev/"

GAR_HD bool proto_is(Str p, char a, char b, char c) {
  return p.n == 3 && (p.p[0] | 0x20) == a && (p.p[1] | 0x20) == b && (p.p[2] | 0x20) == c;
}

GAR_HD void classify_object(const DevTables &T, const Work &W, u32 i) {
  const gar_objects &o = T.o;
  u32 kind = o.obj_kind[i];
  u32 dv = 0;
  bool has_lbtype = false, has_ingclass = false;
  gar_str r53 = 0, name = 0, tags = 0, listen = 0;
  bool has_listen = false;
  for (u32 k = o.obj_ann_begin[i]; k < o.obj_ann_begin[i + 1]; k++) {
    Str key = mkstr(o.slab, o.ann_key[k]);
    gar_str vref = o.ann_val[k];
    if (HAS_PREFIX_LIT(key, ANN_PREFIX)) {
      Str t = substr(key, sizeof(ANN_PREFIX) - 1, key.n - (u32)(sizeof(ANN_PREFIX) - 1));
      if (STREQ_LIT(t, "global-accelerator-managed")) {
        dv |= GAR_DV_GA_MANAGED;
      } else if (STREQ_LIT(t, "route53-hostname")) {
        dv |= GAR_DV_R53_ANNOTATED;
        r53 = vref;
      } else if (STREQ_LIT(t, "client-ip-preservation")) {
        if (STREQ_LIT(mkstr(o.slab, vref), "true")) dv |= GAR_DV_IP_PRESERVE;
        else dv &= ~(u32)GAR_DV_IP_PRESERVE;
      } else if (STREQ_LIT(t, "global-accelerator-name")) {
        dv |= OBJ_HAS_NAME_ANN;
        name = vref;
      } else if (STREQ_LIT(t, "global-accelerator-tags")) {
        dv |= OBJ_HAS_TAGS_ANN;
        tags = vref;
      } else if (STREQ_LIT(t, "ip-address-type")) {
        Str v = mkstr(o.slab, vref);
        if (STREQ_LIT(v, "ipv4") || STREQ_LIT(v, "IPV4")) dv |= GAR_DV_IPV4;
        else dv &= ~(u32)GAR_DV_IPV4;
      }
    } else if (STREQ_LIT(key, "service.beta.kubernetes.io/aws-load-balancer-type")) {
      has_lbtype = true;
    } else if (STREQ_LIT(key, "kubernetes.io/ingress.class")) {
      has_ingclass = true;
    } else if (STREQ_LIT(key, "alb.ingress.kubernetes.io/listen-ports")) {
      has_listen = true;
      listen = vref;
    }
  }
  if (kind == GAR_KIND_SERVICE) {
    bool lbsvc = o.obj_spec_type[i] == GAR_SVC_LOADBALANCER && (has_lbtype || (o.obj_flags[i] & GAR_OBJ_HAS_LB_CLASS));
    if (lbsvc) dv |= GAR_DV_GA_ELIGIBLE | GAR_DV_R53_ELIGIBLE;
    bool udp = false;
    for (u32 p = o.obj_port_begin[i]; p < o.obj_port_begin[i + 1]; p++) {
      Str pr = mkstr(o.slab, o.port_proto[p]);
      if (proto_is(pr, 'u', 'd', 'p')) udp = true;
      else if (proto_is(pr, 't', 'c', 'p')) udp = false;
    }
    if (udp) dv |= GAR_DV_PROTO_UDP;
  } else {
    bool alb = has_ingclass;
    if ((o.obj_flags[i] & GAR_OBJ_HAS_INGRESS_CLASS) && STREQ_LIT(mkstr(o.slab, o.obj_ingress_class[i]), "alb")) alb = true;
    if (alb) dv |= GAR_DV_GA_ELIGIBLE;
    dv |= GAR_DV_R53_ELIGIBLE;
    if (has_listen) dv |= GAR_DV_PORTS_FROM_ANN;
  }
  if (!object_key_ok(T, i)) dv |= OBJ_KEY_BAD;
  const u64 okh = (dv & OBJ_KEY_BAD) ? 0 : key_hash_kinded(kind, object_key(T, i));
  W.okey_hash[i] = okh;
  if (!(dv & OBJ_KEY_BAD)) ix_count(W.hist[IX_OBJ], okh);
  W.derived[i] = dv;
  W.ann_r53[i] = r53;
  W.ann_name[i] = name;
  W.ann_tags[i] = tags;
  W.ann_listen[i] = listen;
}


GAR_HD u32 name_dash_id(Str s) {
  u32 last = GAR_NONE;
  for (u32 i = 0; i < s.n; i += 8) {
    u64 w = load_word(s, i);
    u64 pad = s.n - i < 8 ? ~lowmask(s.n - i) & 0x8080808080808080ull : 0;
    if (w & 0x8080808080808080ull) return 0;
    u64 dash = swar_eq_exact(w, '-') & ~pad;
    u64 ok = swar_in_range(w, '0', '9') | swar_in_range(w, 'A', 'Z') | swar_in_range(w, 'a', 'z') | swar_eq_exact(w, '_') | dash | pad;
    if (ok != 0x8080808080808080ull) return 0;
    if (dash) last = i + ((63 - clz64(dash)) >> 3);
  }
  if (last == GAR_NONE || last < 1 || last + 1 >= s.n) return 0;
  return last;
}

GAR_HD u8 tokenise_str(Str h, u64 base, gar_str *name_out, gar_str *region_out) {
  u8 code;
  gar_str name = 0, region = 0;
  u32 d1 = find_byte(h, 0, '.');
  u32 d2 = d1 < h.n ? find_byte(h, d1 + 1, '.') : h.n;
  u32 d3 = d2 < h.n ? find_byte(h, d2 + 1, '.') : h.n;
  if (d1 >= h.n) {
    code = GAR_TOK_PANIC;
  } else if (!(STREQ_LIT(h, "amazonaws.com") || HAS_SUFFIX_LIT(h, ".amazonaws.com"))) {
    code = GAR_TOK_NOT_AWS;
  } else if (HAS_SUFFIX_LIT(h, ".elb.amazonaws.com")) {
    Str sub = substr(h, 0, d1);
    region = GAR_STR(base + d1 + 1, d2 - d1 - 1);
    if (HAS_PREFIX_LIT(sub, "internal-")) {
      u32 g = name_dash_id(substr(sub, 9, sub.n - 9));
// ... 177 lines not shown

struct OwnRange {
  u32 pos, end;
};
GAR_HD OwnRange own_accs(const Work &W, u32 i) {
  const u32 s = 2 * W.obj_canon[i];
  return OwnRange{W.own_begin[s], W.own_begin[s + 1]};
}
GAR_HD OwnRange own_vals(const Work &W, u32 i) {
  const u32 s = 2 * W.obj_canon[i] + 1;
  return OwnRange{W.own_begin[s], W.own_begin[s + 1]};
}

struct OwnerIter {
  Cursor c;
  Str key;
};
GAR_HD OwnerIter owner_open(const Work &W, u64 key_hash, Str key) { return OwnerIter{idx_open(W.ix_owner, key_hash), key}; }
GAR_HD u32 owner_next(const DevTables &T, const Work &W, u32 kind, OwnerIter &it) {
  IdxEntry e;
  while (idx_next(W.ix_owner, it.c, &e)) {
    if ((((e.a0 & ACC_OWNER_INGRESS) != 0) ? 1u : 0u) != kind) continue;
    if (streq(mkstr(T.a.slab, e.s0), it.key)) return e.row;
  }
  return GAR_NONE;
}

GAR_HD u32 find_by_hostname(const DevTables &T, const Work &W, Str hostname, u32 *first, gar_str *first_dns) {
  Cursor c = idx_open(W.ix_thost, key_hash_str(hostname));
  u32 n = 0;
  *first = GAR_NONE;
  IdxEntry e;
  while (idx_next(W.ix_thost, c, &e)) {
    if (!streq(mkstr(T.a.slab, e.s0), hostname)) continue;
    if (n == 0) {
      *first = e.row;
      *first_dns = e.s1;
    }
    if (++n >= 2) break;
  }
  return n;
}

GAR_HD bool zone_len_possible(const Work &W, u32 n) {
  u32 b = n < 255 ? n : 255;
  return (W.zone_len_mask[b >> 6] >> (b & 63)) & 1ull;
}
GAR_HD u32 find_hosted_zone(const DevTables &T, const Work &W, Str hostname) {
  Str t = hostname;
  for (;;) {
    if (t.n == 0) return GAR_NONE;
    if (zone_len_possible(W, t.n)) {
      Cursor c = idx_open(W.ix_zone, key_hash_str(t));
      IdxEntry e;
      while (idx_next(W.ix_zone, c, &e)) {
        Str zn = mkstr(T.a.slab, e.s0);
        if (zn.n == t.n + 1 && streq(substr(zn, 0, t.n), t)) return e.row;
      }
    }
    u32 k = find_byte(t, 0, '.');
    if (k >= t.n) return GAR_NONE;
    t = substr(t, k + 1, t.n - k - 1);
  }
}

GAR_HD bool record_name_matches(Str name, Str hostname) {
  u32 w = GAR_NONE;
  for (u32 k = find_byte(name, 0, '\\'); k + 4 <= name.n; k = find_byte(name, k + 1, '\\'))
    if (name.p[k + 1] == '0' && name.p[k + 2] == '5' && name.p[k + 3] == '2') {
      w = k;
      break;
    }
  if (w == GAR_NONE) return name.n == hostname.n + 1 && name.p[name.n - 1] == '.' && streq(substr(name, 0, hostname.n), hostname);
  if (name.n - 3 != hostname.n + 1) return false;
  if (name.p[name.n - 1] != '.') return false;
  if (w >= hostname.n || hostname.p[w] != '*') return false;
  if (!streq(substr(name, 0, w), substr(hostname, 0, w))) return false;
  u32 tail = hostname.n - w - 1;
  return streq(substr(name, w + 4, tail), substr(hostname, w + 1, tail));
}


GAR_HD Cursor cursor_none() { return Cursor{0, 0, 0}; }
GAR_HD Cursor u_open(const HashIdx &ix, bool active, u64 h) { return active ? idx_open(ix, h) : cursor_none(); }

GAR_HD bool u_bucket_step(const HashIdx &ix, bool searching, Cursor &c, IdxEntry *e) {
  bool step = searching && c.pos < c.end;
  if (step) {
    *e = load_entry(ix.ent + c.pos++);
    return e->tag == c.tag;
  }
  return false;
}
#define U_BUCKET_LOOP(searching_expr, cur) for (; GAR_ANY((searching_expr) && (cur).pos < (cur).end);)

GAR_HD u32 u_find_lb(const DevTables &T, const Work &W, bool active, Str region, Str name, u32 *state) {
  u64 h = hmix(u_hash(active, region), u_hash(active, name));
  Cursor c = u_open(W.ix_lb, active, h);
  u32 found = GAR_NONE;
  U_BUCKET_LOOP(found == GAR_NONE, c) {
    IdxEntry e;
    bool hit = u_bucket_step(W.ix_lb, found == GAR_NONE, c, &e);
    bool eq = u_streq(hit, mkstr(T.a.slab, e.s0), name);
    eq = u_streq(eq, mkstr(T.a.slab, e.s1), region);
    if (eq) {
      found = e.row;
      *state = e.a0;
    }
  }
  return found;
}

GAR_HD u32 u_find_by_hostname(const DevTables &T, const Work &W, bool active, Str hostname, u32 *first, gar_str *first_dns) {
  Cursor c = u_open(W.ix_thost, active, u_hash(active, hostname));
  u32 n = 0;
  *first = GAR_NONE;
  U_BUCKET_LOOP(n < 2, c) {
    IdxEntry e;
    bool hit = u_bucket_step(W.ix_thost, n < 2, c, &e);
    if (u_streq(hit, mkstr(T.a.slab, e.s0), hostname)) {
      if (n == 0) {
        *first = e.row;
        *first_dns = e.s1;
      }
      n++;
    }
  }
  return n;
}

GAR_HD u32 u_find_hosted_zone(const DevTables &T, const Work &W, bool active, Str hostname) {
  Str t = hostname;
  u32 zone = GAR_NONE;
  bool walking = active;
  for (;;) {
    bool round = walking && t.n != 0;
    if (!GAR_ANY(round)) break;
    bool probe = round && zone_len_possible(W, t.n);
    Cursor c = u_open(W.ix_zone, probe, u_hash(probe, t));
    U_BUCKET_LOOP(zone == GAR_NONE, c) {
      IdxEntry e;
      bool hit = u_bucket_step(W.ix_zone, zone == GAR_NONE, c, &e);
      Str zn = mkstr(T.a.slab, e.s0);
      hit = hit && zn.n == t.n + 1;
      if (u_streq(hit, substr(zn, 0, hit ? t.n : 0), t)) zone = e.row;
    }
    u32 k = u_find_byte(round && zone == GAR_NONE, t, 0, '.');
    if (round) {
      if (zone != GAR_NONE || k >= t.n) walking = false;
      else t = substr(t, k + 1, t.n - k - 1);
    }
  }
  return zone;
}

GAR_HD u32 u_first_alias_a(const DevTables &T, const Work &W, bool active, u32 zone, Str name, gar_str *alias_dns) {
  Cursor c = u_open(W.ix_alias, active, hmix((u64)zone + 0x100, u_hash(active, name)));
  u32 found = GAR_NONE;
  U_BUCKET_LOOP(found == GAR_NONE, c) {
    IdxEntry e;
    bool hit = u_bucket_step(W.ix_alias, found == GAR_NONE, c, &e);
    hit = hit && e.a0 == zone && e.a1 == GAR_RR_A;
    if (u_streq(hit, mkstr(T.a.slab, e.s0), name)) {
      found = e.row;
      *alias_dns = e.s1;
    }
  }
  return found;
}

GAR_HD bool u_record_name_matches(bool active, Str name, Str hostname) {
  u32 bs = u_find_byte(active, name, 0, '\\');
  bool plain = active && bs >= name.n;
  bool shape = plain && name.n == hostname.n + 1 && name.p[name.n - 1] == '.';
  bool eq = u_streq(shape, substr(name, 0, shape ? hostname.n : 0), hostname);
  if (active && !plain) eq = record_name_matches(name, hostname);
  return eq;
}


struct OpSink {
  gar_op *out;
  u32 n;
  u32 cap;
  GAR_HD void put(u32 head, u32 obj, u32 sub, u32 a0, u32 a1, u32 a2) {
    if (out && n < cap) {
      gar_op o;
      o.head = head;
      o.obj = obj;
      o.sub = sub;
      o.a0 = a0;
      o.a1 = a1;
      o.a2 = a2;
      out[n] = o;
    }
    n++;
  }
};


struct PortList {
  const i32 *p;
  u32 n;
};
GAR_HD PortList desired_ports(const DevTables &T, const Work &W, u32 i) {
  if (W.derived[i] & GAR_DV_PORTS_FROM_ANN) {
    u32 b = W.dport_begin[i], e = W.dport_begin[i + 1];
    if (e > W.dport_cap) b = e = 0;
    return PortList{W.dports + b, e - b};
  }
  u32 b = T.o.obj_port_begin[i];
  return PortList{T.o.port_number + b, T.o.obj_port_begin[i + 1] - b};
}

GAR_HD bool ports_changed(PortList l, PortList d) {
  u32 nmin = l.n < d.n ? l.n : d.n;
  u32 pre = 0;
  while (pre < nmin && l.p[pre] == d.p[pre]) pre++;
  u32 suf = 0;
  while (suf < nmin - pre && l.p[l.n - 1 - suf] == d.p[d.n - 1 - suf]) suf++;
  u32 ml = l.n - pre - suf, md = d.n - pre - suf;
  for (u32 x = 0; x < ml + md; x++) {
    i32 px = x < ml ? l.p[pre + x] : d.p[pre + (x - ml)];
    u32 cnt = 0;
    for (u32 y = 0; y < l.n && cnt < 2; y++) cnt += (l.p[y] == px);
    for (u32 y = 0; y < d.n && cnt < 2; y++) cnt += (d.p[y] == px);
    if (cnt <= 1) return true;
  }
  return false;
}

GAR_HD bool accel_name_matches(const DevTables &T, const Work &W, u32 i, u32 kind, Str acc_name) {
  if (W.derived[i] & OBJ_HAS_NAME_ANN) {
    Str n = mkstr(T.o.slab, W.ann_name[i]);
    if (n.n != 0) return streq(n, acc_name);
  }
  Str ns = mkstr(T.o.slab, T.o.obj_ns[i]), nm = mkstr(T.o.slab, T.o.obj_name[i]);
  if (acc_name.n != 7 + 1 + ns.n + 1 + nm.n) return false;
  const u64 res = kind == GAR_KIND_SERVICE ? 0x2d65636976726573ull  : 0x2d73736572676e69ull ;
  if (ld64u(acc_name.p) != res) return false;
  if (acc_name.p[8 + ns.n] != '-') return false;
  return streq(substr(acc_name, 8, ns.n), ns) && streq(substr(acc_name, 9 + ns.n, nm.n), nm);
}

GAR_HD Str actual_tag(const DevTables &T, u32 acc, Str key) {
  Str v{T.a.slab, 0};
  for (u32 t = T.a.acc_tag_begin[acc]; t < T.a.acc_tag_begin[acc + 1]; t++)
    if (streq(mkstr(T.a.slab, T.a.tag_key[t]), key)) v = mkstr(T.a.slab, T.a.tag_val[t]);
  return v;
}

struct TagPiece {
  Str key, val;
  bool ok;
};
GAR_HD TagPiece tag_piece(Str piece) {
  u32 eq = find_byte(piece, 0, '=');
  TagPiece t;
  t.ok = eq < piece.n && find_byte(piece, eq + 1, '=') >= piece.n;
  if (t.ok) {
    t.key = substr(piece, 0, eq);
    t.val = substr(piece, eq + 1, piece.n - eq - 1);
  } else {
    t.key = t.val = Str{piece.p, 0};
  }
  return t;
}
GAR_HD bool next_piece(Str all, u32 *pos, Str *piece) {
  if (*pos > all.n) return false;
  u32 b = *pos;
  u32 k = find_byte(all, b, ',');
  *piece = substr(all, b, k - b);
  *pos = k + 1;
  return true;
}

GAR_HD bool accelerator_tags_changed(const DevTables &T, const Work &W, u32 i, u32 kind, u32 acc, Str lb_dns) {
  const gar_actual &A = T.a;
  bool user_managed = false, user_owner = false, user_thost = false;
  if (W.derived[i] & OBJ_HAS_TAGS_ANN) {
    Str tags = mkstr(T.o.slab, W.ann_tags[i]);
    u32 pos = 0;
    Str piece;
    while (next_piece(tags, &pos, &piece)) {
      TagPiece tp = tag_piece(piece);
      if (!tp.ok) continue;
      if (STREQ_LIT(tp.key, TAG_MANAGED)) user_managed = true;
      else if (STREQ_LIT(tp.key, TAG_OWNER)) user_owner = true;
      else if (STREQ_LIT(tp.key, TAG_THOST)) user_thost = true;
      bool overridden = false;
      u32 pos2 = pos;
      Str piece2;
      while (next_piece(tags, &pos2, &piece2)) {
        TagPiece t2 = tag_piece(piece2);
        if (t2.ok && streq(t2.key, tp.key)) {
          overridden = true;
          break;
        }
      }
      if (overridden) continue;
      if (!streq(actual_tag(T, acc, tp.key), tp.val)) return true;
    }
  }
  u32 fl = W.acc_flags[acc];
  if (!user_managed && !STREQ_LIT(mkstr(A.slab, W.acc_managed[acc]), "true")) return true;
  if (!user_owner) {
    bool ok = (fl & ACC_OWNER_KEYED) && (((fl & ACC_OWNER_INGRESS) ? 1u : 0u) == kind) && streq(mkstr(A.slab, W.acc_owner_key[acc]), object_key(T, i));
    if (!ok) return true;
  }
  if (!user_thost && !streq(mkstr(A.slab, W.acc_thost[acc]), lb_dns)) return true;
  return false;
}

GAR_HD void put_delete_chain(const DevTables &T, OpSink &s, u32 obj, u32 kind, u32 acc) {
  const gar_actual &A = T.a;
  u32 lb = A.acc_lis_begin[acc], le = A.acc_lis_begin[acc + 1];
  u32 lis = GAR_NONE, eg = GAR_NONE;
  if (le - lb == 1) {
    lis = lb;
    u32 eb = A.lis_eg_begin[lis], ee = A.lis_eg_begin[lis + 1];
    if (ee - eb == 1) eg = eb;
// ... 134 lines not shown
    const bool later = go && prev_lb != GAR_NONE;
    if (later) ga_later_step(T, W, i, kind, okey, jb, j, lb, prev_lb, pending, s, &ev);
    go = go && !later;
    OwnRange oc = go ? own_accs(W, i) : OwnRange{0, 0};
    Str lb_arn = go ? mkstr(A.slab, A.lb_arn[lb]) : Str{A.slab, 0};
    u32 nacc = 0;
    for (;;) {
      bool a = go && !stop && oc.pos < oc.end;
      if (!GAR_ANY(a)) break;
      u32 acc = a ? W.own[oc.pos++].row : GAR_NONE;
      if (a) nacc++;
      AccDigest d;
      d.flags = 0;
      if (a) d = W.acc_digest[acc];
      if (u_accelerator_changed(T, W, a, i, dv, kind, acc, d, okey, lb_dns)) s.put(GAR_OP_HEAD(GAR_OP_GA_UPDATE_ACCEL, GAR_CTRL_GA, kind), i, j, acc, lb, GAR_NONE);
      u32 eg = GAR_NONE;
      if (a) {
        if (d.flags & ACCD_LIS_MANY) {
          result = GAR_STATUS(GAR_ST_ERR_RETRY, GAR_D_TOO_MANY_LISTENERS, ev);
          stop = true;
        } else if (d.flags & ACCD_LIS_NONE) {
          s.put(GAR_OP_HEAD(GAR_OP_GA_CREATE_LISTENER, GAR_CTRL_GA, kind), i, j, acc, GAR_NONE, GAR_NONE);
          s.put(GAR_OP_HEAD(GAR_OP_GA_CREATE_EG, GAR_CTRL_GA, kind), i, j, acc, GAR_NONE, lb);
        } else {
          u32 lis = d.lis;
          bool want_udp = kind == GAR_KIND_SERVICE && (dv & GAR_DV_PROTO_UDP);
          bool changed = ((d.flags & ACCD_LIS_UDP) != 0) != want_udp;
          if (!changed) {
            PortList want = desired_ports(T, W, i);
            if (d.n_ports <= 2 && want.n == d.n_ports && (d.n_ports < 1 || want.p[0] == d.port0) && (d.n_ports < 2 || (want.p[1] == d.port1 && d.port0 != d.port1))) changed = false;
            else changed = ports_changed(PortList{A.pr_from + d.pr_begin, d.n_ports == 0xFFFF ? A.lis_pr_begin[lis + 1] - d.pr_begin : d.n_ports}, want);
          }
          if (changed) s.put(GAR_OP_HEAD(GAR_OP_GA_UPDATE_LISTENER, GAR_CTRL_GA, kind), i, j, acc, lis, GAR_NONE);
          if (d.flags & ACCD_EG_MANY) {
            result = GAR_STATUS(GAR_ST_ERR_RETRY, GAR_D_TOO_MANY_EGS, ev);
            stop = true;
          } else if (d.flags & ACCD_EG_NONE) {
            s.put(GAR_OP_HEAD(GAR_OP_GA_CREATE_EG, GAR_CTRL_GA, kind), i, j, acc, lis, lb);
          } else {
            eg = d.eg;
          }
        }
      }
      bool contains = false;
      u32 nep = eg != GAR_NONE ? (d.n_eps == 0xFFFF ? A.eg_ep_begin[eg + 1] - d.ep_begin : d.n_eps) : 0;
      for (u32 x = 0;; x++) {
        bool more = !contains && x < nep;
        if (!GAR_ANY(more)) break;
        gar_str id = more ? (x == 0 ? d.ep0 : A.ep_id[d.ep_begin + x]) : 0;
        if (u_streq(more, mkstr(A.slab, id), lb_arn)) contains = true;
      }
      if (eg != GAR_NONE && !contains) s.put(GAR_OP_HEAD(GAR_OP_GA_UPDATE_EG, GAR_CTRL_GA, kind), i, j, acc, eg, lb);
    }
    if (go && !stop && nacc == 0) {
      s.put(GAR_OP_HEAD(GAR_OP_GA_CREATE_CHAIN, GAR_CTRL_GA, kind), i, j, lb, GAR_NONE, GAR_NONE);
      ev |= GAR_EV_CREATED;
      pending = true;
    }
    if ((go || later) && !stop) prev_lb = lb;
  }
  if (ensure && !stop) result = GAR_STATUS(GAR_ST_OK, 0, ev);
  return result;
}

GAR_HD void ga_later_step(const DevTables &T, const Work &W, u32 i, u32 kind, Str okey, u32 jb, u32 j, u32 lb, u32 prev_lb, bool pending, OpSink &s, u32 *ev) {
  const gar_actual &A = T.a;
  bool keep_visible, user_thost;
  user_tag_effects(T, W, i, kind, okey, &keep_visible, &user_thost);
  if (!keep_visible) {
    s.put(GAR_OP_HEAD(GAR_OP_GA_CREATE_CHAIN, GAR_CTRL_GA, kind), i, j, lb, GAR_NONE, GAR_NONE);
    *ev |= GAR_EV_CREATED;
    return;
  }
  Str lb_arn = mkstr(A.slab, A.lb_arn[lb]);
  const bool dns_differs = !user_thost && !streq(mkstr(A.slab, A.lb_dns[lb]), mkstr(A.slab, A.lb_dns[prev_lb]));
  const bool arn_differs = !streq(lb_arn, mkstr(A.slab, A.lb_arn[prev_lb]));
  if (pending) {
    if (dns_differs) s.put(GAR_OP_HEAD(GAR_OP_GA_UPDATE_ACCEL, GAR_CTRL_GA, kind), i, j, GAR_PENDING, lb, GAR_NONE);
    if (arn_differs) s.put(GAR_OP_HEAD(GAR_OP_GA_UPDATE_EG, GAR_CTRL_GA, kind), i, j, GAR_PENDING, GAR_PENDING, lb);
  }
  const OwnRange ar = own_accs(W, i);
  for (u32 p = ar.pos; p < ar.end; p++) {
    const u32 acc = W.own[p].row;
    if (dns_differs) s.put(GAR_OP_HEAD(GAR_OP_GA_UPDATE_ACCEL, GAR_CTRL_GA, kind), i, j, acc, lb, GAR_NONE);
    const AccDigest d = W.acc_digest[acc];
    const bool created = (d.flags & (ACCD_LIS_NONE | ACCD_EG_NONE)) != 0;
    bool replaced = created;
    for (u32 jp = 0; jp < j && !replaced; jp++) {
      if (W.tok_code[jb + jp] > GAR_TOK_NLB) continue;
      u32 st;
      u32 lbp = find_lb(T, W, mkstr(T.o.slab, W.tok_region[jb + jp]), mkstr(T.o.slab, W.tok_name[jb + jp]), &st);
      if (lbp != GAR_NONE && !eg_contains(T, d, mkstr(A.slab, A.lb_arn[lbp]))) replaced = true;
    }
    const bool contains = replaced ? !arn_differs : eg_contains(T, d, lb_arn);
    if (!contains) s.put(GAR_OP_HEAD(GAR_OP_GA_UPDATE_EG, GAR_CTRL_GA, kind), i, j, acc, created ? GAR_PENDING : d.eg, lb);
  }
}


struct OwnedHit {
  u32 v, rec, zone;
  gar_str name;
};
GAR_HD OwnedHit owned_hit(const IdxEntry &e) { return OwnedHit{e.row, e.a0, e.a1 & 0x3FFFFFFFu, e.s1}; }
struct OwnedList {
  const IdxEntry *e;
  u32 n;
};
GAR_HD OwnedList owned_list(const Work &W, u32 i) {
  const OwnRange r = own_vals(W, i);
  return OwnedList{W.own + r.pos, r.end - r.pos};
}
GAR_HD OwnedHit owned_get(const DevTables &, const Work &, const OwnedList &o, u32 k) { return owned_hit(load_entry(o.e + k)); }
constexpr u32 OWNED_CACHE = 8;
struct Owned {
  OwnedHit hit[OWNED_CACHE];
  u32 n;
  u64 okh;
  u32 kind;
  Str key;
};
GAR_HD bool owned_match(const DevTables &T, const IdxEntry &e, u32 kind, Str key) {
  return (e.a1 >> 31) == kind && streq(mkstr(T.a.slab, e.s0), key);
}
GAR_HD void owned_collect(const DevTables &T, const Work &W, u64 okh, u32 kind, Str key, Owned &o) {
  o.n = 0;
  o.okh = okh;
  o.kind = kind;
  o.key = key;
  Cursor c = idx_open(W.ix_val, okh);
  IdxEntry e;
  while (idx_next(W.ix_val, c, &e)) {
    if (!owned_match(T, e, kind, key)) continue;
    if (o.n < OWNED_CACHE) o.hit[o.n] = owned_hit(e);
    o.n++;
  }
}
GAR_HD OwnedHit owned_get(const DevTables &T, const Work &W, const Owned &o, u32 k) {
  if (k < OWNED_CACHE) return o.hit[k];
  Cursor c = idx_open(W.ix_val, o.okh);
  IdxEntry e;
  u32 seen = 0;
  OwnedHit h{GAR_NONE, GAR_NONE, GAR_NONE, 0};
  while (idx_next(W.ix_val, c, &e)) {
    if (!owned_match(T, e, o.kind, o.key)) continue;
    if (seen++ == k) {
      h = owned_hit(e);
      break;
    }
  }
  return h;
}

GAR_HD u32 first_alias_a(const DevTables &T, const Work &W, u32 zone, Str name, u64 name_hash, gar_str *alias_dns) {
  Cursor c = idx_open(W.ix_alias, key_hash_zoned_h(zone, name_hash));
  IdxEntry e;
  while (idx_next(W.ix_alias, c, &e)) {
    if (e.a0 != zone || e.a1 != GAR_RR_A) continue;
    if (streq(mkstr(T.a.slab, e.s0), name)) {
      *alias_dns = e.s1;
      return e.row;
    }
  }
  return GAR_NONE;
}
GAR_HD u32 next_alias_any(const DevTables &T, const Work &W, u32 zone, Str name, u32 after ) {
  Cursor c = idx_open(W.ix_alias, key_hash_zoned(zone, name));
  IdxEntry e;
  while (idx_next(W.ix_alias, c, &e)) {
    if (after != GAR_NONE && e.row <= after) continue;
    if (e.a0 != zone) continue;
    if (streq(mkstr(T.a.slab, e.s0), name)) return e.row;
  }
  return GAR_NONE;
}

template <class OwnedT>
GAR_HD void r53_cleanup(const DevTables &T, const Work &W, u32 obj, u32 kind, const OwnedT &ow, OpSink &s) {
  const gar_actual &A = T.a;
  u32 head = GAR_OP_HEAD(GAR_OP_R53_DELETE_RECORD, GAR_CTRL_R53, obj == GAR_NONE ? 0 : kind);
  u32 k = 0;
  while (k < ow.n) {
    u32 zone = owned_get(T, W, ow, k).zone;
    u32 kend = k;
    while (kend < ow.n && owned_get(T, W, ow, kend).zone == zone) kend++;
    u32 last = GAR_NONE;
    for (;;) {
      u32 best = GAR_NONE, best_v = GAR_NONE;
      for (u32 x = k; x < kend; x++) {
        OwnedHit h = owned_get(T, W, ow, x);
        u32 r = next_alias_any(T, W, zone, mkstr(A.slab, h.name), last);
        if (r != GAR_NONE && (best == GAR_NONE || r < best)) {
          best = r;
          best_v = h.v;
        }
      }
      if (best == GAR_NONE) break;
      s.put(head, obj, 0, zone, best, best_v);
      last = best;
    }
    for (u32 x = k; x < kend; x++) {
      OwnedHit h = owned_get(T, W, ow, x);
      s.put(head, obj, 1, zone, h.rec, h.v);
    }
    k = kend;
  }
}

GAR_HD bool piece_seen_before(Str all, Str hn) {
  u32 pos = 0;
  Str piece;
  while (next_piece(all, &pos, &piece)) {
    if (piece.p >= hn.p) return false;
    if (streq(piece, hn)) return true;
  }
  return false;
}

GAR_HD u32 r53_reconcile(const DevTables &T, const Work &W, u32 i, bool valid, OpSink &s) {
  const gar_objects &o = T.o;
  const gar_actual &A = T.a;
  u32 result = GAR_STATUS(GAR_ST_IGNORED, 0, 0);
  u32 kind = 0, jb = 0, nj = 0;
  Str hostnames{T.o.slab, 0};
  bool ensure = false;
  OwnedList ow{W.own, 0};
  if (valid) {
    u32 dv = W.derived[i];
    if (dv & GAR_DV_R53_ELIGIBLE) {
      kind = o.obj_kind[i];
      if (!(dv & GAR_DV_R53_ANNOTATED)) {
        r53_cleanup(T, W, i, kind, owned_list(W, i), s);
        result = GAR_STATUS(GAR_ST_OK, 0, GAR_EV_DELETED);
      } else {
        ensure = true;
        hostnames = mkstr(o.slab, W.ann_r53[i]);
        jb = o.obj_lbi_begin[i];
        nj = o.obj_lbi_begin[i + 1] - jb;
      }
    }
  }
  u32 ev = 0;
  bool stop = false;
  bool have_prev = false;
  Str prev_acc_dns{A.slab, 0};
  for (u32 j = 0;; j++) {
    bool act = ensure && !stop && j < nj;
    if (!GAR_ANY(act)) break;
    bool probe = false;
    Str lbhost{o.slab, 0};
    if (act) {
      u32 code = W.tok_code[jb + j];
      if (code == GAR_TOK_PANIC) {
        result = GAR_STATUS(GAR_ST_PANIC, 0, ev);
        stop = true;
      } else if (code == GAR_TOK_NOT_AWS) {
      } else if (code >= GAR_TOK_ERR_NOT_ELB) {
        result = GAR_STATUS(GAR_ST_ERR_RETRY, GAR_D_NOT_ELB + (code - GAR_TOK_ERR_NOT_ELB), ev);
        stop = true;
      } else {
        probe = true;
        lbhost = mkstr(o.slab, o.lbi_hostname[jb + j]);
      }
    }
    u32 acc = GAR_NONE;
    gar_str acc_dns_ref = 0;
    u32 nacc = u_find_by_hostname(T, W, probe, lbhost, &acc, &acc_dns_ref);
    bool go = false;
    if (probe) {
      if (nacc > 1) {
        result = GAR_STATUS(GAR_ST_REQUEUE_60S, GAR_D_ACCEL_MANY, ev);
        stop = true;
      } else if (nacc == 0) {
        result = GAR_STATUS(GAR_ST_REQUEUE_60S, GAR_D_ACCEL_NONE, ev);
        stop = true;
      } else {
        go = true;
      }
    }
    Str acc_dns = go ? mkstr(A.slab, acc_dns_ref) : Str{A.slab, 0};
    if (go) ow = owned_list(W, i);
    bool created = false;
    u32 pos = 0, k = 0;
    for (;;) {
      bool more = go && !stop && pos <= hostnames.n;
      if (!GAR_ANY(more)) break;
      u32 comma = u_find_byte(more, hostnames, pos, ',');
      Str hn = more ? substr(hostnames, pos, comma - pos) : Str{o.slab, 0};
      pos = comma + 1;
      u32 zone = u_find_hosted_zone(T, W, more, hn);
      if (more && zone == GAR_NONE) {
        result = GAR_STATUS(GAR_ST_ERR_RETRY, GAR_D_NO_HOSTED_ZONE, ev);
        stop = true;
        more = false;
      }
      u32 rec = GAR_NONE;
      gar_str rec_alias = 0;
      for (u32 x = 0;; x++) {
        bool has = more && x < ow.n;
        if (!GAR_ANY(has)) break;
        Str nm{A.slab, 0};
        bool inzone = false;
        if (has) {
          OwnedHit h = owned_get(T, W, ow, x);
          inzone = h.zone == zone;
          if (inzone) nm = mkstr(A.slab, h.name);
        }
        bool cand = u_record_name_matches(inzone, nm, hn);
        gar_str al = 0;
        u32 r = u_first_alias_a(T, W, cand, zone, nm, &al);
        if (cand && r != GAR_NONE && (rec == GAR_NONE || r < rec)) {
          rec = r;
          rec_alias = al;
        }
      }
      bool have = more && rec != GAR_NONE;
      Str al = have ? mkstr(A.slab, rec_alias) : Str{A.slab, 0};
      bool shape = have && al.n == acc_dns.n + 1 && al.p[al.n - 1] == '.';
      bool same = u_streq(shape, substr(al, 0, shape ? acc_dns.n : 0), acc_dns);
      if (more) {
        if (!piece_seen_before(hostnames, hn)) {
          if (!have_prev) {
            if (rec == GAR_NONE) {
              s.put(GAR_OP_HEAD(GAR_OP_R53_CREATE, GAR_CTRL_R53, kind), i, GAR_R53_SUB(j, k), zone, acc, GAR_NONE);
              created = true;
            } else if (!same) {
              s.put(GAR_OP_HEAD(GAR_OP_R53_UPSERT_A, GAR_CTRL_R53, kind), i, GAR_R53_SUB(j, k), zone, acc, rec);
            }
          } else if (!streq(acc_dns, prev_acc_dns)) {
            s.put(GAR_OP_HEAD(GAR_OP_R53_UPSERT_A, GAR_CTRL_R53, kind), i, GAR_R53_SUB(j, k), zone, acc, rec == GAR_NONE ? GAR_PENDING : rec);
          }
        }
        k++;
      }
    }
    if (go && !stop && created) ev |= GAR_EV_CREATED;
    if (go && !stop) {
      have_prev = true;
      prev_acc_dns = acc_dns;
    }
  }
  if (ensure && !stop) result = GAR_STATUS(GAR_ST_OK, 0, ev);
  return result;
}


GAR_HD void link_value_alias(const DevTables &T, const Work &W, u32 v) {
  u32 row = GAR_NONE;
  gar_str dns = 0;
  if (W.val_cls[v] != VAL_NOT_OWNER) {
    u32 rec = W.val_rec[v];
    row = first_alias_a(T, W, W.rec_zone[rec], mkstr(T.a.slab, T.a.rec_name[rec]), W.rec_name_hash[rec], &dns);
  }
  ValLink l;
  l.alias_row = row;
  l.pad = 0;
  l.alias_dns = dns;
  W.val_link[v] = l;
}

GAR_HD void r53_prepare(const DevTables &T, const Work &W, u32 i, u32 t, bool valid, u32 *status) {
  const gar_objects &o = T.o;
  u32 mode = R53_MODE_DONE, st = GAR_STATUS(GAR_ST_IGNORED, 0, 0), npairs = 0;
  bool probe = false;
  Str lbhost{o.slab, 0}, hostnames{o.slab, 0};
  if (valid) {
    u32 dv = W.derived[i];
    if (dv & GAR_DV_R53_ELIGIBLE) {
      u32 jb = o.obj_lbi_begin[i], nj = o.obj_lbi_begin[i + 1] - jb;
      if (!(dv & GAR_DV_R53_ANNOTATED) || nj > 1) {
        mode = R53_MODE_OBJECT;
      } else if (nj == 0) {
        st = GAR_STATUS(GAR_ST_OK, 0, 0);
      } else {
        u32 code = W.tok_code[jb];
        if (code == GAR_TOK_PANIC) st = GAR_STATUS(GAR_ST_PANIC, 0, 0);
        else if (code == GAR_TOK_NOT_AWS) st = GAR_STATUS(GAR_ST_OK, 0, 0);
        else if (code >= GAR_TOK_ERR_NOT_ELB) st = GAR_STATUS(GAR_ST_ERR_RETRY, GAR_D_NOT_ELB + (code - GAR_TOK_ERR_NOT_ELB), 0);
        else {
          probe = true;
          lbhost = mkstr(o.slab, o.lbi_hostname[jb]);
          hostnames = mkstr(o.slab, W.ann_r53[i]);
        }
      }
    }
  }
  u32 acc = GAR_NONE;
  gar_str acc_dns = 0;
  u32 nacc = u_find_by_hostname(T, W, probe, lbhost, &acc, &acc_dns);
  bool go = false;
  if (probe) {
    if (nacc > 1) st = GAR_STATUS(GAR_ST_REQUEUE_60S, GAR_D_ACCEL_MANY, 0);
    else if (nacc == 0) st = GAR_STATUS(GAR_ST_REQUEUE_60S, GAR_D_ACCEL_NONE, 0);
    else go = true;
  }
  u32 pos = 0;
  for (;;) {
    bool more = go && pos <= hostnames.n;
    if (!GAR_ANY(more)) break;
    u32 comma = u_find_byte(more, hostnames, pos, ',');
    if (more) {
      npairs++;
      pos = comma + 1;
    }
  }
  if (go) mode = R53_MODE_PAIRS;
  if (valid) {
    W.r53_mode[i] = (u8)mode;
    W.r53_acc[i] = acc;
    W.r53_acc_dns[i] = acc_dns;
    W.pair_begin[t] = npairs;
    if (mode == R53_MODE_DONE) status[t] = st;
  }
}

GAR_HD void r53_fill_pairs(const DevTables &T, const Work &W, u32 i, u32 t) {
  if (W.r53_mode[i] != R53_MODE_PAIRS) return;
  gar_str ref = W.ann_r53[i];
  Str hostnames = mkstr(T.o.slab, ref);
  u32 p = W.pair_begin[t], pos = 0, np = 0;
  u32 st[8], ln[8];
  Str piece;
  while (next_piece(hostnames, &pos, &piece)) {
    if (p >= W.pair_cap) break;
    W.pair_obj[p] = i;
    W.pair_hn[p] = GAR_STR(GAR_STR_OFF(ref) + (u64)(piece.p - hostnames.p), piece.n);
    bool repeat = false;
    for (u32 q = 0; q < np && q < 8 && !repeat; q++) repeat = ln[q] == piece.n && streq(substr(hostnames, st[q], ln[q]), piece);
    if (!repeat && np > 8) repeat = piece_seen_before(hostnames, piece);
    W.pair_code[p] = repeat ? (u8)PAIR_REPEAT : (u8)PAIR_IN_SYNC;
    if (np < 8) {
      st[np] = (u32)(piece.p - hostnames.p);
      ln[np] = piece.n;
    }
    np++;
    p++;
  }
}

GAR_HD void r53_pair(const DevTables &T, const Work &W, u32 p, bool valid) {
  const gar_actual &A = T.a;
  u32 i = 0;
  Str hn{T.o.slab, 0};
  valid = valid && W.pair_code[p] != PAIR_REPEAT;
  if (valid) {
    i = W.pair_obj[p];
    hn = mkstr(T.o.slab, W.pair_hn[p]);
  }
  u32 zone = u_find_hosted_zone(T, W, valid, hn);
  bool live = valid && zone != GAR_NONE;
  u32 rec = GAR_NONE;
  gar_str rec_alias = 0;
  OwnRange c = live ? own_vals(W, i) : OwnRange{0, 0};
  for (; GAR_ANY(c.pos < c.end);) {
    IdxEntry e;
    bool mine = false;
    if (c.pos < c.end) {
      e = load_entry(W.own + c.pos++);
      mine = (e.a1 & 0x3FFFFFFFu) == zone;
    }
    Str nm = mine ? mkstr(A.slab, e.s1) : Str{A.slab, 0};
    bool plain = mine && !(e.a1 & VALNAME_HAS_BACKSLASH);
    bool shape = plain && nm.n == hn.n + 1 && nm.p[nm.n - 1] == '.';
    bool match = u_streq(shape, substr(nm, 0, shape ? hn.n : 0), hn);
    if (mine && !plain) match = record_name_matches(nm, hn);
    if (match && e.tag != GAR_NONE && (rec == GAR_NONE || e.tag < rec)) {
      rec = e.tag;
      rec_alias = e.s0;
    }
  }
  bool have = live && rec != GAR_NONE;
  Str acc_dns = have ? mkstr(A.slab, W.r53_acc_dns[i]) : Str{A.slab, 0};
  Str al = have ? mkstr(A.slab, rec_alias) : Str{A.slab, 0};
  bool shape = have && al.n == acc_dns.n + 1 && al.p[al.n - 1] == '.';
  bool same = u_streq(shape, substr(al, 0, shape ? acc_dns.n : 0), acc_dns);
  if (valid) {
    u32 code = !live ? PAIR_NO_ZONE : rec == GAR_NONE ? PAIR_CREATE : same ? PAIR_IN_SYNC : PAIR_UPSERT;
    W.pair_code[p] = (u8)code;
    W.pair_zone[p] = zone;
    W.pair_rec[p] = rec;
  }
}

GAR_HD u32 r53_combine(const DevTables &T, const Work &W, u32 i, u32 t, bool valid, u32 prev_status, OpSink &s) {
  u32 mode = valid ? W.r53_mode[i] : R53_MODE_DONE;
  u32 st = prev_status;
  bool slow = mode == R53_MODE_OBJECT;
  if (GAR_ANY(slow)) {
    u32 r = r53_reconcile(T, W, i, slow, s);
    if (slow) st = r;
  }
  if (mode == R53_MODE_PAIRS) {
    u32 kind = T.o.obj_kind[i], acc = W.r53_acc[i];
    bool created = false, stop = false;
    u32 k = 0;
    for (u32 p = W.pair_begin[t]; p < W.pair_begin[t + 1] && p < W.pair_cap && !stop; p++, k++) {
      u32 code = W.pair_code[p];
      if (code == PAIR_NO_ZONE) {
        st = GAR_STATUS(GAR_ST_ERR_RETRY, GAR_D_NO_HOSTED_ZONE, 0);
        stop = true;
      } else if (code == PAIR_CREATE) {
        s.put(GAR_OP_HEAD(GAR_OP_R53_CREATE, GAR_CTRL_R53, kind), i, GAR_R53_SUB(0, k), W.pair_zone[p], acc, GAR_NONE);
        created = true;
      } else if (code == PAIR_UPSERT) {
        s.put(GAR_OP_HEAD(GAR_OP_R53_UPSERT_A, GAR_CTRL_R53, kind), i, GAR_R53_SUB(0, k), W.pair_zone[p], acc, W.pair_rec[p]);
      }
    }
    if (!stop) st = GAR_STATUS(GAR_ST_OK, 0, created ? GAR_EV_CREATED : 0);
  }
  return st;
}

// ... 209 lines not shown
```

aws-global-accelerator-controller_b200/csrc/gar_shard.h:

```cpp
#pragma once

#include "gar_pipeline.h"

#if defined(__CUDA_ARCH__)
#define GAR_ATOMIC_OR(p, v) atomicOr((p), (v))
#else
#define GAR_ATOMIC_OR(p, v) (*(p) |= (v))
#endif

constexpr int SH_MAX_RANKS = GAR_SHARD_MAX_RANKS;
constexpr int SH_MAX_SEGS = 2 * SH_MAX_RANKS;
enum ShLevel { L_OBJ, L_ANN, L_LBI, L_PORT, L_ACC, L_TAG, L_LIS, L_PR, L_EG, L_EP, L_REC, L_VAL, L_ZONE, L_LB, L_STUB, L_STUBTAG, L_PROBE, L_NLEVELS };
static_assert(2 * L_NLEVELS + 1 <= GAR_SHARD_META_WORDS, "meta row too small");
constexpr int SH_MAX_STR = 4, SH_MAX_U8 = 3, SH_MAX_U32 = 1, SH_MAX_CHILD = 3;
enum { SH_ARENA_PLAN = 0, SH_ARENA_DIR = 1, SH_ARENA_HOME = 2 };
constexpr u32 SH_DROP = 255;
constexpr u32 SH_FOLLOW = 254;

struct LevelSchema {
  int n_str, n_u8, n_u32, has_gid, n_child;
  int child[SH_MAX_CHILD];
};
static const LevelSchema SH_SCHEMA[L_NLEVELS] = {
     {2, 3, 1, 1, 3, {L_ANN, L_LBI, L_PORT}},
// ... 12 lines not shown
     {4, 1, 0, 1, 0, {0, 0, 0}},
     {2, 1, 0, 1, 1, {L_STUBTAG, 0, 0}},
     {2, 0, 0, 0, 0, {0, 0, 0}},
     {1, 0, 1, 0, 0, {0, 0, 0}},
};

struct LevelLayout {
  u64 str[SH_MAX_STR], u8c[SH_MAX_U8], u32c[SH_MAX_U32], gid, cnt[SH_MAX_CHILD], slab, end;
};
inline u64 sh_align(u64 x) { return (x + 15) & ~(u64)15; }
inline LevelLayout level_layout(int lvl, u64 base, u64 n, u64 slab_bytes) {
  const LevelSchema &S = SH_SCHEMA[lvl];
  LevelLayout L{};
  u64 p = base;
  for (int c = 0; c < S.n_str; c++) { L.str[c] = p; p = sh_align(p + 8 * n); }
  for (int c = 0; c < S.n_u8; c++) { L.u8c[c] = p; p = sh_align(p + n); }
  for (int c = 0; c < S.n_u32; c++) { L.u32c[c] = p; p = sh_align(p + 4 * n); }
  if (S.has_gid) { L.gid = p; p = sh_align(p + 4 * n); }
  for (int c = 0; c < S.n_child; c++) { L.cnt[c] = p; p = sh_align(p + 4 * n); }
  L.slab = p;
  p = sh_align(p + slab_bytes);
  L.end = p;
  return L;
}
inline u64 blob_bytes(const u64 *meta) {
  u64 p = 0;
  for (int l = 0; l < L_NLEVELS; l++) p = level_layout(l, p, meta[l], meta[L_NLEVELS + l]).end;
  return p;
}


struct LevelSrc {
  const gar_str *str[SH_MAX_STR];
  const u8 *u8c[SH_MAX_U8];
  const u32 *u32c[SH_MAX_U32];
  const u32 *gid;
  u32 gid_base;
  const u32 *child_begin[SH_MAX_CHILD];
  const u8 *child_dest[SH_MAX_CHILD];
  const u8 *slab;
  u32 n;
};
struct LevelPlan {
  u32 *sel;
  u32 *m;
  u32 cap;
  u32 *row_off;
  u32 *slab_scan;
  u32 *slab_off;
  u32 *cnt[SH_MAX_CHILD];
  u32 multi;
};

GAR_HD u32 sh_pad8(u32 len) { return (len + 7u) & ~7u; }
GAR_HD u32 shard_of(u64 h, u32 n_ranks) { return (u32)(xx_avalanche(h + 0x9E3779B97F4A7C15ull) >> 33) % n_ranks; }
GAR_HD u64 directory_key(u8 code, Str host, Str region, Str name) { return code <= GAR_TOK_NLB ? key_hash_lb(region, name) : gar_hash(host); }
GAR_HD u32 dest_of(u32 j, const u32 *row_off, u32 n_ranks) {
  u32 d = 0;
  while (d + 1 < n_ranks && j >= row_off[d + 1]) d++;
  return d;
}


struct FShKeyObj {
  Work W;
  u32 G;
  u32 *keys, *vals;
  GAR_HD void operator()(u32 i) const {
    keys[i] = shard_of(W.okey_hash[i], G);
    vals[i] = i;
  }
};
struct FShObjKey {
  DevTables T;
  gar_str *key;
  u32 *ns_len;
  GAR_HD void operator()(u32 i) const {
    gar_str ns = T.o.obj_ns[i];
    key[i] = GAR_STR(GAR_STR_OFF(ns), GAR_STR_LEN(ns) + 1 + GAR_STR_LEN(T.o.obj_name[i]));
    ns_len[i] = (u32)GAR_STR_LEN(ns);
  }
};
struct FShKeyLb {
  DevTables T;
  u32 G;
  u32 *keys, *vals;
  GAR_HD void operator()(u32 i) const {
    keys[i] = shard_of(key_hash_lb(mkstr(T.a.slab, T.a.lb_region[i]), mkstr(T.a.slab, T.a.lb_name[i])), G);
    vals[i] = i;
  }
};
struct FShKeyAcc {
  Work W;
  u32 G;
  u32 *keys, *vals;
  GAR_HD void operator()(u32 a) const {
    u32 fl = W.acc_flags[a];
    keys[a] = ((fl & ACC_MINE) && (fl & ACC_OWNER_KEYED)) ? shard_of(W.acc_owner_hash[a], G) : SH_DROP;
    vals[a] = a;
  }
};
struct FShKeyStub {
  DevTables T;
  Work W;
  u32 G;
  u32 *keys, *vals;
  GAR_HD void operator()(u32 a) const {
    u32 k = SH_DROP;
    if (W.acc_flags[a] & ACC_MINE) {
      gar_str th = W.acc_thost[a], name, region;
      Str h = mkstr(T.a.slab, th);
      u8 code = tokenise_str(h, GAR_STR_OFF(th), &name, &region);
      k = shard_of(directory_key(code, h, mkstr(T.a.slab, region), mkstr(T.a.slab, name)), G);
    }
    keys[a] = k;
    vals[a] = a;
  }
};
struct FShKeyProbe {
  DevTables T;
  Work W;
  const u32 *lbi_obj;
  u32 G;
  u32 *keys, *vals, *home;
  GAR_HD void operator()(u32 l) const {
    Str h = mkstr(T.o.slab, T.o.lbi_hostname[l]);
    keys[l] = shard_of(directory_key(W.tok_code[l], h, mkstr(T.o.slab, W.tok_region[l]), mkstr(T.o.slab, W.tok_name[l])), G);
    vals[l] = l;
    home[l] = shard_of(W.okey_hash[lbi_obj[l]], G);
  }
};
struct FShStubTagKeep {
  DevTables T;
  u8 *keep;
  GAR_HD void operator()(u32 t) const {
    Str k = mkstr(T.a.slab, T.a.tag_key[t]);
    keep[t] = (STREQ_LIT(k, TAG_MANAGED) || STREQ_LIT(k, TAG_THOST) || STREQ_LIT(k, TAG_CLUSTER)) ? (u8)SH_FOLLOW : (u8)SH_DROP;
  }
};
struct FShValDest {
  Work W;
  u32 G;
  u8 *val_dest;
  GAR_HD void operator()(u32 v) const { val_dest[v] = W.val_cls[v] == VAL_NOT_OWNER ? (u8)SH_DROP : (u8)shard_of(W.val_key_hash[v], G); }
};
struct FShRecMask {
  DevTables T;
  Work W;
  const u8 *val_dest;
  u32 *mask;
  GAR_HD void operator()(u32 v) const {
    u32 d = val_dest[v];
    if (d == SH_DROP) return;
    u32 rec = W.val_rec[v], zone = W.rec_zone[rec];
    const u32 bit = 1u << d;
    if (!(mask[rec] & bit)) GAR_ATOMIC_OR(&mask[rec], bit);
    Str name = mkstr(T.a.slab, T.a.rec_name[rec]);
    Cursor c = idx_open(W.ix_alias, key_hash_zoned_h(zone, W.rec_name_hash[rec]));
    IdxEntry e;
    while (idx_next(W.ix_alias, c, &e)) {
      if (e.a0 != zone || e.row == rec || !streq(mkstr(T.a.slab, e.s0), name)) continue;
      if (!(mask[e.row] & bit)) GAR_ATOMIC_OR(&mask[e.row], bit);
    }
  }
};
struct FShIota {
  u32 *keys, *vals;
  u32 key;
  GAR_HD void operator()(u32 i) const {
    keys[i] = key;
    vals[i] = i;
  }
};


struct FShSelBounds {
  const u32 *keys;
  u32 n, G;
  u32 *row_off, *m;
  GAR_HD void operator()(u32 d) const {
    u32 lo = 0, hi = n;
    while (lo < hi) {
      u32 mid = (lo + hi) >> 1;
      if (keys[mid] < d) lo = mid + 1;
      else hi = mid;
    }
    row_off[d] = lo;
    if (d == G) *m = lo;
  }
};
constexpr u32 SH_MASK_TILE = 32;
struct FShMaskCount {
  const u32 *mask;
  u32 n, G, T;
  u32 *counts;
  GAR_HD void operator()(u32 t) const {
    u32 c[SH_MAX_RANKS];
    for (int d = 0; d < SH_MAX_RANKS; d++) c[d] = 0;
    u32 r1 = (t + 1) * SH_MASK_TILE < n ? (t + 1) * SH_MASK_TILE : n;
    for (u32 r = t * SH_MASK_TILE; r < r1; r++) {
      u32 m = mask[r];
      for (int d = 0; d < SH_MAX_RANKS; d++) c[d] += (m >> d) & 1u;
    }
    for (int d = 0; d < SH_MAX_RANKS; d++)
      if ((u32)d < G) counts[(size_t)d * T + t] = c[d];
  }
};
struct FShMaskFill {
  const u32 *mask;
  u32 n, G, T;
  const u32 *scanned;
  u32 *sel;
  GAR_HD void operator()(u32 t) const {
    u32 pos[SH_MAX_RANKS];
    for (int d = 0; d < SH_MAX_RANKS; d++) pos[d] = (u32)d < G ? scanned[(size_t)d * T + t] : 0;
    u32 r1 = (t + 1) * SH_MASK_TILE < n ? (t + 1) * SH_MASK_TILE : n;
    for (u32 r = t * SH_MASK_TILE; r < r1; r++) {
      u32 m = mask[r];
      for (int d = 0; d < SH_MAX_RANKS; d++)
        if ((m >> d) & 1u) sel[pos[d]++] = r;
    }
  }
};
struct FShMaskBounds {
  const u32 *scanned;
  u32 G, T;
  u32 *row_off, *m;
  GAR_HD void operator()(u32 d) const {
    u32 v = scanned[(size_t)d * T];
    row_off[d] = v;
    if (d == G) *m = v;
  }
};
struct FShChildFill {
  LevelSrc src;
  int link;
  LevelPlan P;
  u32 G;
  u32 *child_sel;
  GAR_HD void operator()(u32 j) const {
    if (j >= *P.m) return;
    u32 p = P.sel[j], b0 = src.child_begin[link][p], b1 = src.child_begin[link][p + 1];
    u32 pos = P.cnt[link][j];
    const u8 *cd = src.child_dest[link];
    if (cd) {
      u32 d = dest_of(j, P.row_off, G);
      for (u32 ch = b0; ch < b1; ch++)
        if (cd[ch] == d || cd[ch] == SH_FOLLOW) child_sel[pos++] = ch;
    } else {
      for (u32 ch = b0; ch < b1; ch++) child_sel[pos++] = ch;
    }
  }
};
struct FShDerivedBounds {
  const u32 *parent_row_off, *scanned;
  u32 G;
  u32 *out_off, *out_m;
  GAR_HD void operator()(u32 d) const {
    u32 v = scanned[parent_row_off[d]];
    out_off[d] = v;
    if (d == G && out_m) *out_m = v;
  }
};
struct FShRowSizes {
  LevelSrc src;
  LevelSchema S;
  LevelPlan P;
  u32 G;
  GAR_HD void operator()(u32 j) const {
    u32 cnt[SH_MAX_CHILD] = {0, 0, 0}, bytes = 0;
    if (j < *P.m) {
      u32 p = P.sel[j], d = 0;
      bool need_d = false;
      for (int c = 0; c < SH_MAX_CHILD; c++) need_d |= c < S.n_child && src.child_dest[c] != nullptr;
      if (need_d) d = dest_of(j, P.row_off, G);
      for (int c = 0; c < SH_MAX_CHILD; c++) {
        if (c >= S.n_child) break;
        u32 b0 = src.child_begin[c][p], b1 = src.child_begin[c][p + 1];
        const u8 *cd = src.child_dest[c];
        if (cd) {
          for (u32 ch = b0; ch < b1; ch++) cnt[c] += cd[ch] == d || cd[ch] == SH_FOLLOW;
        } else {
          cnt[c] = b1 - b0;
        }
      }
      for (int c = 0; c < SH_MAX_STR; c++)
        if (c < S.n_str) bytes += sh_pad8((u32)GAR_STR_LEN(src.str[c][p]));
    }
    for (int c = 0; c < SH_MAX_CHILD; c++)
      if (c < S.n_child) P.cnt[c][j] = cnt[c];
    P.slab_scan[j] = bytes;
  }
};


struct PackDst {
  u8 *base[SH_MAX_RANKS];
  LevelLayout lay[SH_MAX_RANKS];
};
constexpr u32 SH_LONG_WORDS = 256;
GAR_HD void sh_copy_words(u64 *dst, const u8 *s, u32 words) {
  if (!words) return;
  uintptr_t a = (uintptr_t)s;
  const u64 *q = (const u64 *)(a & ~(uintptr_t)7);
  const unsigned sh = (unsigned)(a & 7) * 8;
  u64 lo = q[0];
#pragma unroll 4
  for (u32 w = 0; w < words; w++) {
    u64 hi = q[w + 1];
    dst[w] = (lo >> sh) | ((hi << 1) << (63 - sh));
    lo = hi;
  }
}
struct FShPackRows {
  LevelSrc src;
  LevelSchema S;
// ... 705 lines not shown
```

Measured before the change: 181.3 million.

## Precompute per-record alias links with per-zone shared-memory sort instead of global alias index

Replaces the global hashed alias index and its per-lookup probing with a per-zone block kernel. The kernel bitonic-sorts alias hash tags in shared memory and writes, for every record, its first alias, first A-type alias and next alias. Downstream lookups (value resolution, R53 cleanup, shard masks) then become array reads or linked-list walks. Zones that overflow the 4096-entry shared buffer or have long equal-tag runs fall back to a smaller global index sized by a device-reported count, which can trigger an extra retry pass and a host download on first run.

```diff
diff --git a/aws-global-accelerator-controller_b200/csrc/gar_engine.cu b/aws-global-accelerator-controller_b200/csrc/gar_engine.cu
--- a/aws-global-accelerator-controller_b200/csrc/gar_engine.cu
+++ b/aws-global-accelerator-controller_b200/csrc/gar_engine.cu
@@ -104,6 +104,15 @@
   mbar_wait(&bar, 0);
   const u32 i = r0 + threadIdx.x;
   if (i < n) f.run(i, view);
+}
+
+template <class F>
+__global__ void __launch_bounds__(F::kThreads) k_for_each_block(const __grid_constant__ F f) {
+  extern __shared__ __align__(16) u8 block_smem[];
+  for (u32 p = 0; p < F::kPhases; p++) {
+    f(p, blockIdx.x, threadIdx.x, block_smem);
+    __syncthreads();
+  }
 }
 
 template <class F>
@@ -685,6 +694,15 @@
     if (!staged_passes || !(F::kStageByDefault || staged_all)) return for_each(name, n, f);
     stage_begin(name);
     k_for_each_staged<F><<<(n + 255) / 256, 256, 0, stream>>>(f, n);
+    launches++;
+    stage_end();
+  }
+  template <class F>
+  void for_each_block(const char *name, u32 nblocks, const F &f) {
+    static_assert(F::kSmemBytes <= 48 * 1024, "above the default dynamic shared memory limit");
+    if (!nblocks) return;
+    stage_begin(name);
+    k_for_each_block<F><<<nblocks, F::kThreads, F::kSmemBytes, stream>>>(f);
     launches++;
     stage_end();
   }
diff --git a/aws-global-accelerator-controller_b200/csrc/gar_pipeline.h b/aws-global-accelerator-controller_b200/csrc/gar_pipeline.h
--- a/aws-global-accelerator-controller_b200/csrc/gar_pipeline.h
+++ b/aws-global-accelerator-controller_b200/csrc/gar_pipeline.h
@@ -18,7 +18,7 @@
   S_DERIVED, S_OFLAGS, S_OKEY_HASH, S_STAGE_GA, S_STAGE_R53, S_ANN_R53, S_ANN_NAME, S_ANN_TAGS, S_ANN_LISTEN, S_DPORT_BEGIN, S_DPORTS,
   S_TOK_CODE, S_TOK_NAME, S_TOK_REGION,
   S_ACC_FLAGS, S_ACC_OWNER_KEY, S_ACC_OWNER, S_ACC_THOST, S_ACC_MANAGED, S_ACC_OWNER_HASH, S_ACC_THOST_HASH, S_REC_NAME_HASH, S_VAL_KEY_HASH,
-  S_REC_ZONE, S_VAL_REC, S_VAL_CLS, S_VAL_KEY, S_VAL_ORPHAN, S_VAL_LINK, S_ACC_DIGEST,
+  S_REC_ZONE, S_VAL_REC, S_VAL_CLS, S_VAL_KEY, S_VAL_ORPHAN, S_REC_ALIAS_A, S_REC_ALIAS_ANY, S_ALIAS_NEXT, S_ZONE_BIG, S_ACC_DIGEST,
   S_R53_MODE, S_R53_ACC, S_R53_ACC_DNS, S_PAIR_BEGIN, S_PAIR_OBJ, S_PAIR_HN, S_PAIR_CODE, S_PAIR_ZONE, S_PAIR_REC,
   S_IX_LB, S_IX_OWNER = S_IX_LB + 3, S_IX_THOST = S_IX_OWNER + 3, S_IX_ZONE = S_IX_THOST + 3, S_IX_VAL = S_IX_ZONE + 3,
   S_IX_ALIAS = S_IX_VAL + 3, S_IX_OBJ = S_IX_ALIAS + 3, S_IX_OVN = S_IX_OBJ + 3,
@@ -122,7 +122,6 @@
     const u64 nh = gar_hash(nm);
     W.rec_name_hash[r] = nh;
     W.rec_flags[r] = find_byte(nm, 0, '\\') < nm.n ? 1 : 0;
-    if (T.a.rec_has_alias[r]) ix_count(W.hist[IX_ALIAS], key_hash_zoned_h(lo, nh));
     u32 v0 = T.a.rec_val_begin[r], v1 = T.a.rec_val_begin[r + 1];
     if (v1 - v0 > REC_INLINE_VALUES) {
       u32 *list = v1 - v0 > REC_HUGE_VALUES ? huge : big;
@@ -285,7 +284,147 @@
     e->a1 = T.a.rec_type[r];
     e->s0 = T.a.rec_name[r];
     e->s1 = T.a.rec_alias_dns[r];
-    return T.a.rec_has_alias[r] != 0;
+    return T.a.rec_has_alias[r] != 0 && W.zone_big[W.rec_zone[r]];
+  }
+};
+
+GAR_HD u32 next_pow2(u32 x) {
+  u32 p = 1;
+  while (p < x) p <<= 1;
+  return p;
+}
+
+constexpr u32 ZONE_ALIAS_CAP = 4096;
+constexpr u32 ZONE_ALIAS_LOG = 12;
+constexpr u32 ZONE_RUN_CAP = 48;
+struct ZoneAliasSmem {
+  u64 key[ZONE_ALIAS_CAP];
+  u32 n, big;
+};
+struct FZoneAliases {
+  DevTables T;
+  Work W;
+  u32 *big_count;
+  static constexpr u32 kThreads = 512;
+  static constexpr u32 kSortPhases = ZONE_ALIAS_LOG * (ZONE_ALIAS_LOG + 1) / 2;
+  enum : u32 { P_INIT = 0, P_LOAD = 1, P_PAD = 2, P_SORT = 3, P_RUNS = P_SORT + kSortPhases, P_LINK, kPhases };
+  static constexpr u32 kSmemBytes = sizeof(ZoneAliasSmem);
+  GAR_HD void operator()(u32 p, u32 z, u32 tid, void *smem) const {
+    ZoneAliasSmem &S = *(ZoneAliasSmem *)smem;
+    const u32 r0 = T.a.zone_rec_begin[z], r1 = T.a.zone_rec_begin[z + 1];
+    if (p == P_INIT) {
+      if (tid == 0) S.n = S.big = 0;
+    } else if (p == P_LOAD) {
+      for (u32 r = r0 + tid; r < r1; r += kThreads) {
+        if (!T.a.rec_has_alias[r]) continue;
+#if defined(__CUDA_ARCH__)
+        const u32 pos = atomicAdd(&S.n, 1u);
+#else
+        const u32 pos = S.n++;
+#endif
+        if (pos < ZONE_ALIAS_CAP) S.key[pos] = ((u64)hash_tag(key_hash_zoned_h(z, W.rec_name_hash[r])) << 32) | r;
+      }
+    } else if (p == P_PAD) {
+      const u32 n = S.n;
+      if (n <= ZONE_ALIAS_CAP)
+        for (u32 i = n + tid; i < next_pow2(n); i += kThreads) S.key[i] = ~0ull;
+    } else if (p < P_RUNS) {
+      const u32 n = S.n;
+      if (n > ZONE_ALIAS_CAP) return;
+      u32 q = p - P_SORT, lk = 1;
+      while (q >= lk) q -= lk++;
+      const u32 n2 = next_pow2(n), k = 1u << lk, lj = lk - 1 - q, j = 1u << lj;
+      if (k > n2) return;
+      for (u32 t = tid; t < n2 / 2; t += kThreads) {
+        const u32 i = ((t >> lj) << (lj + 1)) | (t & (j - 1)), l = i + j;
+        const u64 a = S.key[i], b = S.key[l];
+        if ((a > b) == ((i & k) == 0)) {
+          S.key[i] = b;
+          S.key[l] = a;
+        }
+      }
+    } else if (p == P_RUNS) {
+      const u32 n = S.n;
+      if (n > ZONE_ALIAS_CAP) return;
+      for (u32 i = tid; i + ZONE_RUN_CAP < n; i += kThreads)
+        if ((S.key[i] >> 32) == (S.key[i + ZONE_RUN_CAP] >> 32)) S.big = 1;
+    } else {
+      const u32 n = S.n;
+      const bool big = n > ZONE_ALIAS_CAP || S.big;
+      if (tid == 0) {
+        W.zone_big[z] = big ? 1 : 0;
+        if (big) GAR_ATOMIC_ADD(big_count, n);
+      }
+      for (u32 r = r0 + tid; r < r1; r += kThreads) {
+        u32 any = GAR_NONE, a = GAR_NONE, next = GAR_NONE;
+        const bool is_alias = T.a.rec_has_alias[r] != 0;
+        if (!big) {
+          const u64 tag = hash_tag(key_hash_zoned_h(z, W.rec_name_hash[r]));
+          u32 lo = 0, hi = n;
+          while (lo < hi) {
+            const u32 mid = (lo + hi) >> 1;
+            if ((S.key[mid] >> 32) < tag) lo = mid + 1;
+            else hi = mid;
+          }
+          const Str nm = mkstr(T.a.slab, T.a.rec_name[r]);
+          for (u32 k = lo; k < n && (S.key[k] >> 32) == tag; k++) {
+            const u32 c = (u32)S.key[k];
+            const bool want_a = a == GAR_NONE && T.a.rec_type[c] == GAR_RR_A, want_next = is_alias && next == GAR_NONE && c > r;
+            if (any != GAR_NONE && !want_a && !want_next) {
+              if (a != GAR_NONE && (!is_alias || next != GAR_NONE)) break;
+              continue;
+            }
+            if (c != r && !streq(mkstr(T.a.slab, T.a.rec_name[c]), nm)) continue;
+            if (any == GAR_NONE) any = c;
+            if (want_a) a = c;
+            if (want_next) next = c;
+          }
+        }
+        W.rec_alias_any[r] = any;
+        W.rec_alias_a[r] = a;
+        W.alias_next[r] = next;
+      }
+    }
+  }
+};
+template <class F>
+struct FBlockSerial {
+  F f;
+  void operator()(u32 b) const {
+    u64 smem[(F::kSmemBytes + 7) / 8];
+    for (u32 p = 0; p < F::kPhases; p++)
+      for (u32 t = 0; t < F::kThreads; t++) f(p, b, t, smem);
+  }
+};
+template <class B, class F>
+auto run_blocks(B &be, const char *name, u32 nblocks, const F &f, int) -> decltype(be.for_each_block(name, nblocks, f)) {
+  return be.for_each_block(name, nblocks, f);
+}
+template <class B, class F>
+void run_blocks(B &be, const char *name, u32 nblocks, const F &f, long) {
+  be.for_each(name, nblocks, FBlockSerial<F>{f});
+}
+
+struct FAliasLinksBig {
+  DevTables T;
+  Work W;
+  GAR_HD void operator()(u32 r) const {
+    const u32 zone = W.rec_zone[r];
+    if (!W.zone_big[zone]) return;
+    const Str nm = mkstr(T.a.slab, T.a.rec_name[r]);
+    u32 any = GAR_NONE, a = GAR_NONE, next = GAR_NONE;
+    const bool is_alias = T.a.rec_has_alias[r] != 0;
+    Cursor c = idx_open(W.ix_alias, key_hash_zoned_h(zone, W.rec_name_hash[r]));
+    IdxEntry e;
+    while (idx_next(W.ix_alias, c, &e)) {
+      if (e.a0 != zone || !streq(mkstr(T.a.slab, e.s0), nm)) continue;
+      if (e.row < any) any = e.row;
+      if (e.a1 == GAR_RR_A && e.row < a) a = e.row;
+      if (is_alias && e.row > r && e.row < next) next = e.row;
+    }
+    W.rec_alias_any[r] = any;
+    W.rec_alias_a[r] = a;
+    W.alias_next[r] = next;
   }
 };
 struct FRowObj {
@@ -471,7 +610,7 @@
     canon(b, ent, lo, m);
   }
 };
-enum FlagWord { FW_BAD_KEYS = 0, FW_IDX_OVERFLOW = 1, FW_NDPORTS = 2, FW_NPAIRS = 3, FW_SEC0 = 4 , FW_WORDS = 16 };
+enum FlagWord { FW_BAD_KEYS = 0, FW_IDX_OVERFLOW = 1, FW_NDPORTS = 2, FW_NPAIRS = 3, FW_SEC0 = 4 , FW_ALIAS_BIG = 9, FW_WORDS = 16 };
 struct FGatherFinal {
   const u32 *src;
   u32 idx[5];
@@ -496,14 +635,6 @@
   u32 *flags;
   GAR_HD void operator()(u32) const { flags[FW_NDPORTS] = *ndports; }
 };
-struct FValueJoins {
-  DevTables T;
-  Work W;
-  GAR_HD void operator()(u32 v) const {
-    link_value_alias(T, W, v);
-    resolve_value(T, W, v);
-  }
-};
 struct FResolveValue {
   DevTables T;
   Work W;
@@ -522,13 +653,12 @@
     e.row = x;
     return e;
   }
-  const u32 v = x - T.a.n_accels, rec = W.val_rec[v];
-  const ValLink l = W.val_link[v];
-  e.tag = l.alias_row;
+  const u32 v = x - T.a.n_accels, rec = W.val_rec[v], alias = W.rec_alias_a[rec];
+  e.tag = alias;
   e.row = v;
   e.a0 = rec;
   e.a1 = W.rec_zone[rec] | ((W.rec_flags[rec] & 1) ? VALNAME_HAS_BACKSLASH : 0u);
-  e.s0 = l.alias_dns;
+  e.s0 = alias != GAR_NONE ? T.a.rec_alias_dns[alias] : 0;
   e.s1 = T.a.rec_name[rec];
   return e;
 }
@@ -809,11 +939,6 @@
   u32 bad_keys;
 };
 
-GAR_HD u32 next_pow2(u32 x) {
-  u32 p = 1;
-  while (p < x) p <<= 1;
-  return p;
-}
 inline int ilog2(u32 p) {
   int b = 0;
   while ((1u << b) < p) b++;
@@ -829,8 +954,9 @@
   explicit Pipeline(B &b, const DevTables &t) : be(b), T(t) {}
 
   template <class RowF>
-  HashIdx build_index(int slot, u32 nrows, u32 load, RowF rowf, u32 *overflow, bool force_radix, CanonHook canon = {}) {
-    u32 nb = next_pow2(nrows / load < 16 ? 16 : nrows / load);
+  HashIdx build_index(int slot, u32 nrows, u32 load, RowF rowf, u32 *overflow, bool force_radix, CanonHook canon = {}, u32 nkeys = 0) {
+    const u32 nk = nkeys ? nkeys : nrows;
+    u32 nb = next_pow2(nk / load < 16 ? 16 : nk / load);
     u32 *keys = (u32 *)be.ensure(S_SORT_KEYS, sizeof(u32) * (size_t)(nrows + 1));
     u32 *vals = (u32 *)be.ensure(S_SORT_VALS, sizeof(u32) * (size_t)(nrows + 1));
     IdxEntry *tmp = (IdxEntry *)be.ensure(S_SORT_TAGS, sizeof(IdxEntry) * (size_t)(nrows + 1));
@@ -900,7 +1026,10 @@
     W.val_orphan = (u8 *)be.ensure(S_VAL_ORPHAN, nval + 1);
     W.val_obj = (u32 *)be.ensure(S_VAL_OBJ, 4 * (size_t)(nval + 1));
     W.acc_obj = (u32 *)be.ensure(S_ACC_OBJ, 4 * (size_t)(nacc + 1));
-    W.val_link = (ValLink *)be.ensure(S_VAL_LINK, sizeof(ValLink) * (size_t)(nval + 1));
+    W.rec_alias_a = (u32 *)be.ensure(S_REC_ALIAS_A, 4 * (size_t)(nrec + 1));
+    W.rec_alias_any = (u32 *)be.ensure(S_REC_ALIAS_ANY, 4 * (size_t)(nrec + 1));
+    W.alias_next = (u32 *)be.ensure(S_ALIAS_NEXT, 4 * (size_t)(nrec + 1));
+    W.zone_big = (u8 *)be.ensure(S_ZONE_BIG, (size_t)T.a.n_zones + 1);
     W.acc_digest = (AccDigest *)be.ensure(S_ACC_DIGEST, sizeof(AccDigest) * (size_t)(nacc + 1));
     W.lb_hash = (u64 *)be.ensure(S_LB_HASH, 8 * (size_t)(T.a.n_lbs + 1));
     W.rec_flags = (u8 *)be.ensure(S_REC_FLAGS, (size_t)nrec + 1);
@@ -932,7 +1061,20 @@
       be.fill32(huge, 0, 1);
       be.for_each_staged("prepare_records", nrec, FPrepareRecord{T, W, big, huge});
       if (nval > REC_INLINE_VALUES) be.for_each("prepare_records", BIG_BLOCKS * 256, FClassifyBigRecords{T, W, big, huge});
-    }
+      link_aliases();
+    }
+  }
+  u32 alias_big_cap = 0;
+  void link_aliases() {
+    run_blocks(be, "zone_aliases", T.a.n_zones, FZoneAliases{T, W, errflag + FW_ALIAS_BIG}, 0);
+    if (!alias_big_cap) return;
+    W.ix_alias = build_index(S_IX_ALIAS, T.a.n_records, 2, FRowAlias{T, W}, errflag + FW_IDX_OVERFLOW, force_radix, {}, alias_big_cap);
+    be.for_each("zone_aliases_big", T.a.n_records, FAliasLinksBig{T, W});
+  }
+  bool alias_cap_short(const u32 *fl) {
+    if (fl[FW_ALIAS_BIG] <= alias_big_cap) return false;
+    alias_big_cap = fl[FW_ALIAS_BIG] + fl[FW_ALIAS_BIG] / 8 + 16;
+    return true;
   }
   struct IxPlan {
     u32 off[IX_N] = {}, nb[IX_N] = {}, rows[IX_N] = {};
@@ -945,8 +1087,8 @@
   IdxEntry *ixa_ent = nullptr;
   u32 ovn_nb = 0;
   void arm_group_a(u32 want_mask) {
-    const u32 rows[IX_N] = {T.a.n_lbs, T.a.n_accels, T.a.n_accels, T.a.n_zones, T.a.n_values, T.a.n_records, T.o.n_objects, 0};
-    const u32 load[IX_N] = {1, 1, 1, 1, 1, 2, 1, 8};
+    const u32 rows[IX_N] = {T.a.n_lbs, T.a.n_accels, T.a.n_accels, T.a.n_zones, T.a.n_values, 0, T.o.n_objects, 0};
+    const u32 load[IX_N] = {1, 1, 1, 1, 1, 1, 1, 8};
     planA = IxPlan{};
     for (int k = 0; k < IX_OVN; k++) {
       planA.want[k] = (want_mask >> k) & 1u;
@@ -978,18 +1120,17 @@
     be.fill32(ixa_multi, 0, 1);
     const IxPlan &P = planA;
     auto n = [&](int k) { return P.want[k] ? P.rows[k] : 0u; };
-    be.for_each_multi("idx_place", {n(IX_LB), n(IX_THOST), n(IX_ZONE), n(IX_ALIAS), n(IX_OBJ), P.total_nb},
+    be.for_each_multi("idx_place", {n(IX_LB), n(IX_THOST), n(IX_ZONE), n(IX_OBJ), P.total_nb},
                       placer(IX_LB, FRowLb{T, W}), placer(IX_THOST, FRowThost{T, W}), placer(IX_ZONE, FRowZone{T}),
-                      placer(IX_ALIAS, FRowAlias{T, W}), placer(IX_OBJ, FRowObj{T, W}), FIdxMultiList{ixa_begin, ixa_multi});
+                      placer(IX_OBJ, FRowObj{T, W}), FIdxMultiList{ixa_begin, ixa_multi});
     const CanonHook canon = P.want[IX_OBJ] ? canon_hook(P.off[IX_OBJ], P.off[IX_OBJ] + P.nb[IX_OBJ]) : CanonHook{};
     be.for_each_dyn("idx_order", ixa_multi, multi_cap, FIdxOrderMulti{ixa_begin, ixa_ent, ixa_multi, overflow, canon});
     if (P.want[IX_LB]) W.ix_lb = group_a_index(IX_LB);
     if (P.want[IX_THOST]) W.ix_thost = group_a_index(IX_THOST);
     if (P.want[IX_ZONE]) W.ix_zone = group_a_index(IX_ZONE);
-    if (P.want[IX_ALIAS]) W.ix_alias = group_a_index(IX_ALIAS);
     if (P.want[IX_OBJ]) W.ix_obj = group_a_index(IX_OBJ);
   }
-  void resolve_owners(bool link_aliases) {
+  void resolve_owners(const char *name) {
     const u32 n = T.o.n_objects, nacc = T.a.n_accels, nval = T.a.n_values, nseg = 2 * n;
     u32 *overflow = errflag + FW_IDX_OVERFLOW;
     W.own_begin = (u32 *)be.ensure(S_OWN_BEGIN, 4 * (size_t)(nseg + 2));
@@ -1003,8 +1144,7 @@
     } else {
       W.hist[IX_OVN] = IxHist{nullptr, 0};
     }
-    if (link_aliases) be.for_each_multi("value_joins", {nval, nacc}, FValueJoins{T, W}, FResolveAccel{T, W});
-    else be.for_each_multi("resolve_owners", {nval, nacc}, FResolveValue{T, W}, FResolveAccel{T, W});
+    be.for_each_multi(name, {nval, nacc}, FResolveValue{T, W}, FResolveAccel{T, W});
     be.exclusive_scan(W.own_begin, nseg + 1);
     IdxEntry *own = (IdxEntry *)be.ensure(S_OWN_ENT, sizeof(IdxEntry) * ((size_t)nacc + nval + 1));
     if (!force_radix) {
@@ -1052,9 +1192,10 @@
 
   void prepare_route() {
     alloc_work();
-    arm_group_a(1u << IX_ALIAS);
     stage1();
-    finish_group_a();
+    u32 fl[FW_WORDS];
+    be.download(fl, errflag, sizeof(fl));
+    if (alias_cap_short(fl)) link_aliases();
   }
   void prepare_directory() {
     alloc_work();
@@ -1069,9 +1210,9 @@
   u64 ops_cap = 0;
   bool tiny_caps = false;
   int prepare() {
-    const u32 n = T.o.n_objects, nacc = T.a.n_accels, nzone = T.a.n_zones, nrec = T.a.n_records;
+    const u32 n = T.o.n_objects, nacc = T.a.n_accels, nzone = T.a.n_zones;
     alloc_work();
-    if (!force_radix) arm_group_a((1u << IX_LB) | (1u << IX_THOST) | (1u << IX_ZONE) | (1u << IX_ALIAS) | (1u << IX_OBJ));
+    if (!force_radix) arm_group_a((1u << IX_LB) | (1u << IX_THOST) | (1u << IX_ZONE) | (1u << IX_OBJ));
     stage1();
     listen_ports();
 
@@ -1082,10 +1223,9 @@
       W.ix_lb = build_index(S_IX_LB, T.a.n_lbs, 1, FRowLb{T, W}, overflow, true);
       W.ix_thost = build_index(S_IX_THOST, nacc, 1, FRowThost{T, W}, overflow, true);
       W.ix_zone = build_index(S_IX_ZONE, nzone, 1, FRowZone{T}, overflow, true);
-      W.ix_alias = build_index(S_IX_ALIAS, nrec, 2, FRowAlias{T, W}, overflow, true);
       W.ix_obj = build_index(S_IX_OBJ, n, 1, FRowObj{T, W}, overflow, true, canon_hook(0, 0xFFFFFFFFu));
     }
-    resolve_owners(true);
+    resolve_owners("value_joins");
     obj_stale = false;
     owner_indexes = false;
     return GAR_OK;
@@ -1117,7 +1257,7 @@
     owners_stale = true;
   }
   int index_objects() {
-    for (int attempt = 0; attempt < 2; attempt++) {
+    for (int attempt = 0; attempt < 3; attempt++) {
       if (!prepared) prepare();
       else if (obj_stale) prepare_objects();
       prepared = true;
@@ -1126,6 +1266,10 @@
       if (fl[FW_BAD_KEYS]) return GAR_E_INVALID;
       if (fl[FW_IDX_OVERFLOW] && !force_radix) {
         force_radix = true;
+        prepared = false;
+        continue;
+      }
+      if (alias_cap_short(fl)) {
         prepared = false;
         continue;
       }
@@ -1242,14 +1386,14 @@
       u64 sig = 0;
       if (full) {
         sig = hmix(hmix(prepared ? (obj_stale || owners_stale ? 9 : 1) : 2, force_radix ? 3 : 4), hmix(hmix(dport_cap, pair_cap), ops_cap));
-        sig = hmix(sig, hmix(orphan_sweep ? 5 : 6, tiny_caps ? 7 : 8)) | 1;
+        sig = hmix(hmix(sig, hmix(orphan_sweep ? 5 : 6, tiny_caps ? 7 : 8)), alias_big_cap) | 1;
       }
       const int g = full ? be.graph_begin(sig) : 0;
       int rc = GAR_OK;
       if (g != 2) {
         if (!prepared) rc = prepare();
         else if (obj_stale) prepare_objects();
-        if (rc == GAR_OK && owners_stale) resolve_owners(false);
+        if (rc == GAR_OK && owners_stale) resolve_owners("resolve_owners");
         if (rc == GAR_OK) rc = decide();
       }
       prepared = true;
@@ -1263,6 +1407,10 @@
         prepared = false;
         continue;
       }
+      if (alias_cap_short(fl)) {
+        prepared = false;
+        continue;
+      }
       if (fl[FW_NDPORTS] > dport_cap) {
         dport_cap = fl[FW_NDPORTS] + fl[FW_NDPORTS] / 8 + 16;
         prepared = false;
diff --git a/aws-global-accelerator-controller_b200/csrc/gar_rows.h b/aws-global-accelerator-controller_b200/csrc/gar_rows.h
--- a/aws-global-accelerator-controller_b200/csrc/gar_rows.h
+++ b/aws-global-accelerator-controller_b200/csrc/gar_rows.h
@@ -56,11 +56,6 @@
   ACCD_LIS_UDP = 1u << 12,
   ACCD_EG_NONE = 1u << 13, ACCD_EG_MANY = 1u << 14,
 };
-struct alignas(16) ValLink {
-  u32 alias_row, pad;
-  gar_str alias_dns;
-};
-
 enum IxId { IX_LB, IX_OWNER, IX_THOST, IX_ZONE, IX_VAL, IX_ALIAS, IX_OBJ, IX_OVN, IX_N };
 struct IxHist {
   u32 *cnt;
@@ -106,7 +101,10 @@
   gar_str *val_key;
   u64 *val_key_hash;
   u8 *val_orphan;
-  ValLink *val_link;
+  u32 *rec_alias_a;
+  u32 *rec_alias_any;
+  u32 *alias_next;
+  u8 *zone_big;
   u32 acc_guest_from;
   u32 sharded;
   u32 *val_obj;
@@ -590,21 +588,6 @@
     }
   }
   return zone;
-}
-
-GAR_HD u32 u_first_alias_a(const DevTables &T, const Work &W, bool active, u32 zone, Str name, gar_str *alias_dns) {
-  Cursor c = u_open(W.ix_alias, active, hmix((u64)zone + 0x100, u_hash(active, name)));
-  u32 found = GAR_NONE;
-  U_BUCKET_LOOP(found == GAR_NONE, c) {
-    IdxEntry e;
-    bool hit = u_bucket_step(W.ix_alias, found == GAR_NONE, c, &e);
-    hit = hit && e.a0 == zone && e.a1 == GAR_RR_A;
-    if (u_streq(hit, mkstr(T.a.slab, e.s0), name)) {
-      found = e.row;
-      *alias_dns = e.s1;
-    }
-  }
-  return found;
 }
 
 GAR_HD bool u_record_name_matches(bool active, Str name, Str hostname) {
@@ -1045,32 +1028,14 @@
   return h;
 }
 
-GAR_HD u32 first_alias_a(const DevTables &T, const Work &W, u32 zone, Str name, u64 name_hash, gar_str *alias_dns) {
-  Cursor c = idx_open(W.ix_alias, key_hash_zoned_h(zone, name_hash));
-  IdxEntry e;
-  while (idx_next(W.ix_alias, c, &e)) {
-    if (e.a0 != zone || e.a1 != GAR_RR_A) continue;
-    if (streq(mkstr(T.a.slab, e.s0), name)) {
-      *alias_dns = e.s1;
-      return e.row;
-    }
-  }
-  return GAR_NONE;
-}
-GAR_HD u32 next_alias_any(const DevTables &T, const Work &W, u32 zone, Str name, u32 after ) {
-  Cursor c = idx_open(W.ix_alias, key_hash_zoned(zone, name));
-  IdxEntry e;
-  while (idx_next(W.ix_alias, c, &e)) {
-    if (after != GAR_NONE && e.row <= after) continue;
-    if (e.a0 != zone) continue;
-    if (streq(mkstr(T.a.slab, e.s0), name)) return e.row;
-  }
-  return GAR_NONE;
+GAR_HD u32 next_alias_any(const Work &W, u32 rec , u32 after ) {
+  u32 r = W.rec_alias_any[rec];
+  while (r != GAR_NONE && after != GAR_NONE && r <= after) r = W.alias_next[r];
+  return r;
 }
 
 template <class OwnedT>
 GAR_HD void r53_cleanup(const DevTables &T, const Work &W, u32 obj, u32 kind, const OwnedT &ow, OpSink &s) {
-  const gar_actual &A = T.a;
   u32 head = GAR_OP_HEAD(GAR_OP_R53_DELETE_RECORD, GAR_CTRL_R53, obj == GAR_NONE ? 0 : kind);
   u32 k = 0;
   while (k < ow.n) {
@@ -1082,7 +1047,7 @@
       u32 best = GAR_NONE, best_v = GAR_NONE;
       for (u32 x = k; x < kend; x++) {
         OwnedHit h = owned_get(T, W, ow, x);
-        u32 r = next_alias_any(T, W, zone, mkstr(A.slab, h.name), last);
+        u32 r = next_alias_any(W, h.rec, last);
         if (r != GAR_NONE && (best == GAR_NONE || r < best)) {
           best = r;
           best_v = h.v;
@@ -1194,17 +1159,18 @@
         if (!GAR_ANY(has)) break;
         Str nm{A.slab, 0};
         bool inzone = false;
+        IdxEntry e;
+        e.tag = GAR_NONE;
+        e.s0 = 0;
         if (has) {
-          OwnedHit h = owned_get(T, W, ow, x);
-          inzone = h.zone == zone;
-          if (inzone) nm = mkstr(A.slab, h.name);
+          e = load_entry(ow.e + x);
+          inzone = (e.a1 & 0x3FFFFFFFu) == zone;
+          if (inzone) nm = mkstr(A.slab, e.s1);
         }
         bool cand = u_record_name_matches(inzone, nm, hn);
-        gar_str al = 0;
-        u32 r = u_first_alias_a(T, W, cand, zone, nm, &al);
-        if (cand && r != GAR_NONE && (rec == GAR_NONE || r < rec)) {
-          rec = r;
-          rec_alias = al;
+        if (cand && e.tag != GAR_NONE && (rec == GAR_NONE || e.tag < rec)) {
+          rec = e.tag;
+          rec_alias = e.s0;
         }
       }
       bool have = more && rec != GAR_NONE;
@@ -1237,20 +1203,6 @@
   return result;
 }
 
-
-GAR_HD void link_value_alias(const DevTables &T, const Work &W, u32 v) {
-  u32 row = GAR_NONE;
-  gar_str dns = 0;
-  if (W.val_cls[v] != VAL_NOT_OWNER) {
-    u32 rec = W.val_rec[v];
-    row = first_alias_a(T, W, W.rec_zone[rec], mkstr(T.a.slab, T.a.rec_name[rec]), W.rec_name_hash[rec], &dns);
-  }
-  ValLink l;
-  l.alias_row = row;
-  l.pad = 0;
-  l.alias_dns = dns;
-  W.val_link[v] = l;
-}
 
 GAR_HD void r53_prepare(const DevTables &T, const Work &W, u32 i, u32 t, bool valid, u32 *status) {
   const gar_objects &o = T.o;
diff --git a/aws-global-accelerator-controller_b200/csrc/gar_shard.h b/aws-global-accelerator-controller_b200/csrc/gar_shard.h
--- a/aws-global-accelerator-controller_b200/csrc/gar_shard.h
+++ b/aws-global-accelerator-controller_b200/csrc/gar_shard.h
@@ -188,16 +188,11 @@
   GAR_HD void operator()(u32 v) const {
     u32 d = val_dest[v];
     if (d == SH_DROP) return;
-    u32 rec = W.val_rec[v], zone = W.rec_zone[rec];
+    const u32 rec = W.val_rec[v];
     const u32 bit = 1u << d;
     if (!(mask[rec] & bit)) GAR_ATOMIC_OR(&mask[rec], bit);
-    Str name = mkstr(T.a.slab, T.a.rec_name[rec]);
-    Cursor c = idx_open(W.ix_alias, key_hash_zoned_h(zone, W.rec_name_hash[rec]));
-    IdxEntry e;
-    while (idx_next(W.ix_alias, c, &e)) {
-      if (e.a0 != zone || e.row == rec || !streq(mkstr(T.a.slab, e.s0), name)) continue;
-      if (!(mask[e.row] & bit)) GAR_ATOMIC_OR(&mask[e.row], bit);
-    }
+    for (u32 r = W.rec_alias_any[rec]; r != GAR_NONE; r = W.alias_next[r])
+      if (r != rec && !(mask[r] & bit)) GAR_ATOMIC_OR(&mask[r], bit);
   }
 };
 struct FShIota {
```

Result: faster. 192.1 million, median of 6 (+6.0%).
